# zhaozijie2022/LocoTouch

Measured on AMD Instinct MI355X. Metric: env-steps/sec (whole node), TransportTeacher 4096 envs/GPU, higher is better.
Workload: dtype f32

## Files before the change

### locotouch_amd/_abi.py

```python
from __future__ import annotations

import ctypes
import os
import re

_HERE = os.path.dirname(os.path.abspath(__file__))
REPO = os.path.dirname(_HERE)
HEADER = os.path.join(REPO, "include", "lt_env.h")
OBS_NORM_HEADER = os.path.join(REPO, "include", "lt_obs_norm.h")
STUDENT_HEADER = os.path.join(REPO, "include", "lt_student.h")
COLLECT_HEADER = os.path.join(REPO, "include", "lt_collect.h")
LEDGER_HEADER = os.path.join(REPO, "include", "lt_ledger.h")
CNN_TRAIN_HEADER = os.path.join(REPO, "include", "lt_cnn_train.h")
BC_HEADER = os.path.join(REPO, "include", "lt_bc.h")
LSTM_HEADER = os.path.join(REPO, "include", "lt_lstm.h")
MEMORY_HEADER = os.path.join(REPO, "include", "lt_memory.h")
MEMORY_SEQ_HEADER = os.path.join(REPO, "include", "lt_memory_seq.h")
MEMORY_GRU_HEADER = os.path.join(REPO, "include", "lt_memory_gru.h")
POLICY_HEADER = os.path.join(REPO, "include", "lt_policy.h")
LIB_PATH = os.environ.get("LOCOTOUCH_AMD_LIB", os.path.join(_HERE, "_lib", "liblocotouch_env.so"))

_SCALARS = {"int": ctypes.c_int, "int32_t": ctypes.c_int32, "int64_t": ctypes.c_int64, "uint8_t": ctypes.c_uint8,
            "uint32_t": ctypes.c_uint32, "uint64_t": ctypes.c_uint64, "size_t": ctypes.c_size_t, "float": ctypes.c_float,
            "double": ctypes.c_double}
_DECL = re.compile(r"(?:const\s+)?(\w+)\s*((?:\*\s*(?:const\b\s*)?)*)(\w*)\s*((?:\[[^\]]*\]\s*)*)")


def _ctype(decl, structs, opaque, consts, typed, param):
    m = _DECL.fullmatch(decl.strip())
    if not m:
        return None
    base, stars, name, dims = m.groups()
    depth = stars.count("*")
    try:
        dims = [sum(int(t) if t.strip().isdigit() else consts[t.strip()] for t in d.split("+")) for d in re.findall(r"\[([^\]]*)\]", dims)]
    except KeyError:
        return None
    if param and dims:
        depth, dims = depth + 1, dims[1:]
    t = structs.get(base) or _SCALARS.get(base)
    if (t is None and base not in opaque and base not in ("void", "char")) or depth > 2 or (param and dims):
        return None
    if depth == 0 and t is None:
        return None
    if depth == 1 and base == "char":
        t = ctypes.c_char_p
    elif depth == 1:
        t = ctypes.POINTER(t) if t is not None and (typed or base in structs or base == "size_t") else ctypes.c_void_p
    elif depth == 2:
        t = ctypes.POINTER(ctypes.POINTER(t) if typed and t is not None else ctypes.c_void_p)
    for d in reversed(dims):
        t = t * d
    return name, t


def parse_header(text: str, typed: bool = False, structs: dict | None = None, bases: dict | None = None):
    text = re.sub(r"//[^\n]*", "", re.sub(r"/\*.*?\*/", "", text, flags=re.S))
    consts = {m.group(1): int(m.group(2)) for m in re.finditer(r"#define\s+(LT_\w+)\s+\(?(-?\d+)\)?\s*$", text, flags=re.M)}
    for m in re.finditer(r"enum\s+\w+\s*\{(.*?)\};", text, flags=re.S):
        val = -1
        for item in filter(None, (x.strip() for x in m.group(1).split(","))):
            name, _, v = (x.strip() for x in item.partition("="))
            val = int(v, 0) if v else val + 1
            consts[name] = val
    structs, opaque = dict(structs or {}), set(re.findall(r"typedef\s+struct\s+\w+\s+(\w+)\s*;", text))
    for m in re.finditer(r"typedef\s+struct\s+\w+\s*\{(.*?)\}\s*(\w+)\s*;", text, flags=re.S):
        fields = []
        for line in filter(None, (x.strip() for x in m.group(1).split(";"))):
            first, *more = line.split(",")
            base = _DECL.match(first.strip())
            for decl in [first] + [f"{base.group(1) if base else ''} {x}" for x in more]:
                field = _ctype(decl, structs, opaque, consts, typed, param=False)
                if field is None:
                    raise ImportError(f"cannot type member {decl.strip()!r} of {m.group(2)}")
                fields.append(field)
        pyname = "".join(w.capitalize() for w in m.group(2).split("_"))
        structs[m.group(2)] = type(pyname, ((bases or {}).get(m.group(2), ctypes.Structure),), {"_fields_": fields})
    rest = re.sub(r"^[ \t]*#[^\n]*$|typedef\s+struct\b[^;{]*(\{.*?\})?[^;{]*;|enum\s+\w+\s*\{.*?\};|extern\s+\"C\"\s*\{", "", text, flags=re.S | re.M)
    protos = {}
    for stmt in filter(None, (x.strip() for x in rest.split(";"))):
        m = re.fullmatch(r"(.*?)\b(\w+)\s*\(([^()]*)\)", stmt, flags=re.S)
        if not m:
            if stmt == "}":
                continue
            raise ImportError(f"cannot parse declaration {stmt!r}")
        ret, name, args = m.groups()
        res = (None, None) if ret.strip() == "void" else _ctype(ret, structs, opaque, consts, typed, param=False)
        args = [] if args.strip() == "void" else [_ctype(a, structs, opaque, consts, typed, param=True) for a in args.split(",")]
        if res is None or None in args:
            raise ImportError(f"cannot type prototype {name}: {' '.join(stmt.split())!r}")
        protos[name] = (res[1], [t for _, t in args])
    return consts, structs, protos


class _CfgMethods(ctypes.Structure):
    def copy(self) -> "LtCfg":
        new = LtCfg()
        ctypes.memmove(ctypes.byref(new), ctypes.byref(self), ctypes.sizeof(self))
        for attr in ("extra_reward_terms", "extra_termination_terms", "extra_observation_terms", "reward_term_params"):
            if hasattr(self, attr):
                v = getattr(self, attr)
                setattr(new, attr, dict(v) if isinstance(v, dict) else list(v))
        return new

    def to_dict(self) -> dict:
        def py(v):
            return [py(x) for x in v] if hasattr(v, "__len__") else v

        return {name: py(getattr(self, name)) for name, *_ in self._fields_ if not name.startswith("_")}


CONSTS, STRUCTS, SIGNATURES = parse_header(open(HEADER).read(), bases={"lt_cfg": _CfgMethods})
globals().update(CONSTS)
LtCfg, LtView, LtMlpDesc = STRUCTS["lt_cfg"], STRUCTS["lt_view"], STRUCTS["lt_mlp_desc"]
LtRenderView, LtRenderDesc = STRUCTS["lt_render_view"], STRUCTS["lt_render_desc"]
EXPORTS = list(SIGNATURES)
OBS_NORM_SIGNATURES = parse_header(open(OBS_NORM_HEADER).read())[2]
if any(r is not ctypes.c_int for r, _ in OBS_NORM_SIGNATURES.values()) or set(OBS_NORM_SIGNATURES) & set(EXPORTS):
    raise ImportError("include/lt_obs_norm.h: every entry point returns a status and none repeats one of lt_env.h")

VALUE_QUERIES = frozenset({
    "lt_abi_version", "lt_cfg_sizeof", "lt_cfg_num_presets", "lt_cfg_preset_id", "lt_cfg_obs_dim", "lt_cfg_tactile_dim", "lt_last_error",
    "lt_wgrad_splits", "lt_wgrad_ws_floats", "lt_elu_backward_bias_ws_floats", "lt_head_wgrad_ws_floats", "lt_adam_clip_step_ws_floats",
    "lt_elu_backward_bias_nblk", "lt_head_wgrad_nblk", "lt_mlp_backward_blocks", "lt_env_kernel_name", "lt_mlp_kernel_name"})
if not VALUE_QUERIES <= set(EXPORTS) or any(SIGNATURES[n][0] is not ctypes.c_int for n in set(EXPORTS) - VALUE_QUERIES):
    raise ImportError("_abi.VALUE_QUERIES does not match include/lt_env.h: a query it names is gone, or a new entry point returns no status")

STUDENT_CONSTS, _student_structs, STUDENT_SIGNATURES = parse_header(open(STUDENT_HEADER).read(), structs=STRUCTS)
globals().update(STUDENT_CONSTS)
LtStudentDesc, LtStudentParams = _student_structs["lt_student_desc"], _student_structs["lt_student_params"]
STUDENT_VALUE_QUERIES = frozenset({"lt_student_step_launches"})
if (not STUDENT_VALUE_QUERIES <= set(STUDENT_SIGNATURES) or any(r is not ctypes.c_int for r, _ in STUDENT_SIGNATURES.values())
        or set(STUDENT_SIGNATURES) & (set(EXPORTS) | set(OBS_NORM_SIGNATURES))):
    raise ImportError("_abi.STUDENT_VALUE_QUERIES does not match include/lt_student.h, or an entry point there returns no int or repeats "
                      "one of another header")

COLLECT_SIGNATURES = parse_header(open(COLLECT_HEADER).read())[2]
if (any(r is not ctypes.c_int for r, _ in COLLECT_SIGNATURES.values())
        or set(COLLECT_SIGNATURES) & (set(EXPORTS) | set(OBS_NORM_SIGNATURES) | set(STUDENT_SIGNATURES))):
    raise ImportError("include/lt_collect.h: every entry point returns a status and none repeats one of another header")

LEDGER_CONSTS, _, LEDGER_SIGNATURES = parse_header(open(LEDGER_HEADER).read())
if (any(r is not ctypes.c_int for r, _ in LEDGER_SIGNATURES.values())
        or set(LEDGER_SIGNATURES) & (set(EXPORTS) | set(OBS_NORM_SIGNATURES) | set(STUDENT_SIGNATURES) | set(COLLECT_SIGNATURES))):
    raise ImportError("include/lt_ledger.h: every entry point returns a status and none repeats one of another header")

CNN_TRAIN_CONSTS, _cnn_structs, CNN_TRAIN_SIGNATURES = parse_header(open(CNN_TRAIN_HEADER).read())
globals().update(CNN_TRAIN_CONSTS)
LtCnnDesc, LtCnnParams, LtCnnGrads = _cnn_structs["lt_cnn_desc"], _cnn_structs["lt_cnn_params"], _cnn_structs["lt_cnn_grads"]
CNN_TRAIN_VALUE_QUERIES = frozenset({"lt_cnn_launches"})
if (not CNN_TRAIN_VALUE_QUERIES <= set(CNN_TRAIN_SIGNATURES) or any(r is not ctypes.c_int for r, _ in CNN_TRAIN_SIGNATURES.values())
        or set(CNN_TRAIN_SIGNATURES) & (set(EXPORTS) | set(OBS_NORM_SIGNATURES) | set(STUDENT_SIGNATURES) | set(COLLECT_SIGNATURES)
                                        | set(LEDGER_SIGNATURES))):
    raise ImportError("_abi.CNN_TRAIN_VALUE_QUERIES does not match include/lt_cnn_train.h, or an entry point there returns no int or "
                      "repeats one of another header")

BC_CONSTS, _, BC_SIGNATURES = parse_header(open(BC_HEADER).read())
if (any(r is not ctypes.c_int for r, _ in BC_SIGNATURES.values())
        or set(BC_SIGNATURES) & (set(EXPORTS) | set(OBS_NORM_SIGNATURES) | set(STUDENT_SIGNATURES) | set(COLLECT_SIGNATURES)
                                 | set(LEDGER_SIGNATURES) | set(CNN_TRAIN_SIGNATURES))):
    raise ImportError("include/lt_bc.h: every entry point returns a status and none repeats one of another header")

LSTM_SIGNATURES = parse_header(open(LSTM_HEADER).read())[2]
if (any(r is not ctypes.c_int for r, _ in LSTM_SIGNATURES.values())
        or set(LSTM_SIGNATURES) & (set(EXPORTS) | set(OBS_NORM_SIGNATURES) | set(STUDENT_SIGNATURES) | set(COLLECT_SIGNATURES)
                                   | set(LEDGER_SIGNATURES) | set(CNN_TRAIN_SIGNATURES) | set(BC_SIGNATURES))):
    raise ImportError("include/lt_lstm.h: every entry point returns a status and none repeats one of another header")

_, _memory_structs, MEMORY_SIGNATURES = parse_header(open(MEMORY_HEADER).read())
LtMemoryNet = _memory_structs["lt_memory_net"]
if (any(r is not ctypes.c_int for r, _ in MEMORY_SIGNATURES.values())
        or set(MEMORY_SIGNATURES) & (set(EXPORTS) | set(OBS_NORM_SIGNATURES) | set(STUDENT_SIGNATURES) | set(COLLECT_SIGNATURES)
                                     | set(LEDGER_SIGNATURES) | set(CNN_TRAIN_SIGNATURES) | set(BC_SIGNATURES) | set(LSTM_SIGNATURES))):
    raise ImportError("include/lt_memory.h: every entry point returns a status and none repeats one of another header")

_, _memory_seq_structs, MEMORY_SEQ_SIGNATURES = parse_header(open(MEMORY_SEQ_HEADER).read())
LtMemorySeqNet, LtMemorySeqGrad = _memory_seq_structs["lt_memory_seq_net"], _memory_seq_structs["lt_memory_seq_grad"]
MEMORY_SEQ_VALUE_QUERIES = frozenset({"lt_memory_seq_backward_units"})
if (not MEMORY_SEQ_VALUE_QUERIES <= set(MEMORY_SEQ_SIGNATURES) or any(r is not ctypes.c_int for r, _ in MEMORY_SEQ_SIGNATURES.values())
        or set(MEMORY_SEQ_SIGNATURES) & (set(EXPORTS) | set(OBS_NORM_SIGNATURES) | set(STUDENT_SIGNATURES) | set(COLLECT_SIGNATURES)
                                         | set(LEDGER_SIGNATURES) | set(CNN_TRAIN_SIGNATURES) | set(BC_SIGNATURES) | set(LSTM_SIGNATURES)
                                         | set(MEMORY_SIGNATURES))):
    raise ImportError("_abi.MEMORY_SEQ_VALUE_QUERIES does not match include/lt_memory_seq.h, or an entry point there returns no int or "
                      "repeats one of another header")

_, _memory_gru_structs, MEMORY_GRU_SIGNATURES = parse_header(open(MEMORY_GRU_HEADER).read())
LtMemoryGruNet, LtMemoryGruSeqNet, LtMemoryGruSeqGrad = (_memory_gru_structs[k] for k in ("lt_memory_gru_net", "lt_memory_gru_seq_net",
                                                                                           "lt_memory_gru_seq_grad"))
MEMORY_GRU_VALUE_QUERIES = frozenset({"lt_memory_gru_seq_backward_units"})
if (not MEMORY_GRU_VALUE_QUERIES <= set(MEMORY_GRU_SIGNATURES) or any(r is not ctypes.c_int for r, _ in MEMORY_GRU_SIGNATURES.values())
        or set(MEMORY_GRU_SIGNATURES) & (set(EXPORTS) | set(OBS_NORM_SIGNATURES) | set(STUDENT_SIGNATURES) | set(COLLECT_SIGNATURES)
                                         | set(LEDGER_SIGNATURES) | set(CNN_TRAIN_SIGNATURES) | set(BC_SIGNATURES) | set(LSTM_SIGNATURES)
                                         | set(MEMORY_SIGNATURES) | set(MEMORY_SEQ_SIGNATURES))):
    raise ImportError("_abi.MEMORY_GRU_VALUE_QUERIES does not match include/lt_memory_gru.h, or an entry point there returns no int or "
                      "repeats one of another header")

POLICY_CONSTS, _policy_structs, POLICY_SIGNATURES = parse_header(open(POLICY_HEADER).read(), structs=STRUCTS)
globals().update(POLICY_CONSTS)
LtPolicyDesc, LtPolicyMemory = _policy_structs["lt_policy_desc"], _policy_structs["lt_policy_memory"]
POLICY_VALUE_QUERIES = frozenset({"lt_policy_step_launches"})
if (not POLICY_VALUE_QUERIES <= set(POLICY_SIGNATURES) or any(r is not ctypes.c_int for r, _ in POLICY_SIGNATURES.values())
        or set(POLICY_SIGNATURES) & (set(EXPORTS) | set(OBS_NORM_SIGNATURES) | set(STUDENT_SIGNATURES) | set(COLLECT_SIGNATURES)
                                     | set(LEDGER_SIGNATURES) | set(CNN_TRAIN_SIGNATURES) | set(BC_SIGNATURES) | set(LSTM_SIGNATURES)
                                     | set(MEMORY_SIGNATURES) | set(MEMORY_SEQ_SIGNATURES) | set(MEMORY_GRU_SIGNATURES))):
    raise ImportError("_abi.POLICY_VALUE_QUERIES does not match include/lt_policy.h, or an entry point there returns no int or repeats "
                      "one of another header")

_lib = None
_calls: dict = {}


def load() -> ctypes.CDLL:
    global _lib
    if _lib is not None:
        return _lib
    if not os.path.exists(LIB_PATH):
        raise ImportError(f"{LIB_PATH} is missing: run `python -c 'import __graft_entry__ as g; g.build()'` "
                          "(the HIP extension is mandatory, there is no CPU fallback)")
    lib = ctypes.CDLL(LIB_PATH)
    for name, (restype, argtypes) in {**SIGNATURES, **OBS_NORM_SIGNATURES, **STUDENT_SIGNATURES, **COLLECT_SIGNATURES, **LEDGER_SIGNATURES,
                                      **CNN_TRAIN_SIGNATURES, **BC_SIGNATURES, **LSTM_SIGNATURES, **MEMORY_SIGNATURES,
                                      **MEMORY_SEQ_SIGNATURES, **MEMORY_GRU_SIGNATURES, **POLICY_SIGNATURES}.items():
        fn = getattr(lib, name)
        fn.restype, fn.argtypes = restype, argtypes
        if (name not in VALUE_QUERIES and name not in STUDENT_VALUE_QUERIES and name not in CNN_TRAIN_VALUE_QUERIES
                and name not in MEMORY_SEQ_VALUE_QUERIES and name not in MEMORY_GRU_VALUE_QUERIES and name not in POLICY_VALUE_QUERIES):
            _calls[name] = (fn, [ptr if t is ctypes.c_void_p else _ref if issubclass(t, ctypes._Pointer) and issubclass(t._type_, ctypes.Structure)
                                 else None for t in argtypes])
    if lib.lt_cfg_sizeof() != ctypes.sizeof(LtCfg):
        raise ImportError(f"lt_cfg ABI mismatch: C {lib.lt_cfg_sizeof()} vs ctypes {ctypes.sizeof(LtCfg)}")
    if lib.lt_abi_version() != CONSTS["LT_ABI_VERSION"]:
        raise ImportError("lt_env.h / liblocotouch_env.so ABI version mismatch")
    _lib = lib
    return lib


def ptr(x):
    if x is None or isinstance(x, int):
        return ctypes.c_void_p(x or None)
    data_ptr = getattr(x, "data_ptr", None)
    return ctypes.c_void_p(data_ptr()) if data_ptr else x


def _ref(x):
    return ctypes.byref(x) if isinstance(x, ctypes.Structure) else x


def stream(device=None) -> ctypes.c_void_p:
    import torch

    return ctypes.c_void_p(torch.cuda.current_stream(device).cuda_stream)


def ptr_array(tensors):
    return (ctypes.c_void_p * max(1, len(tensors)))(*[None if t is None else t.data_ptr() for t in tensors])


def call(name: str, *args) -> None:
    try:
        fn, conv = _calls[name]
    except KeyError:
        if (name in VALUE_QUERIES or name in STUDENT_VALUE_QUERIES or name in CNN_TRAIN_VALUE_QUERIES or name in MEMORY_SEQ_VALUE_QUERIES
                or name in MEMORY_GRU_VALUE_QUERIES or name in POLICY_VALUE_QUERIES):
            raise TypeError(f"{name} returns a value, not a status: call load().{name}(...)") from None
        if _lib is not None:
            raise
        load()
        fn, conv = _calls[name]
    rc = fn(*[a if c is None else c(a) for c, a in zip(conv, args, strict=True)])
    if rc:
        check(rc, name)


def preset_ids() -> list[str]:
    lib = load()
    return [lib.lt_cfg_preset_id(i).decode() for i in range(lib.lt_cfg_num_presets())]


def preset_cfg(gym_id: str, num_envs: int | None = None, seed: int | None = None) -> LtCfg:
    cfg = LtCfg()
    rc = load().lt_cfg_preset(gym_id.encode(), ctypes.byref(cfg))
    if rc != 0:
        raise KeyError(f"unknown task {gym_id!r}; registered: {preset_ids()}")
    if num_envs is not None:
        cfg.num_envs = int(num_envs)
    if seed is not None:
        cfg.seed = int(seed)
    return cfg


def default_cfg(task: int, num_envs: int | None = None, seed: int | None = None) -> LtCfg:
    cfg = LtCfg()
    rc = load().lt_cfg_default(task, ctypes.byref(cfg))
    if rc != 0:
        raise ValueError(f"lt_cfg_default({task}) failed: {rc}")
    if num_envs is not None:
        cfg.num_envs = num_envs
    if seed is not None:
        cfg.seed = seed
    return cfg


def check(rc: int, what: str) -> None:
    if rc != 0:
        err = load().lt_last_error()
        raise RuntimeError(f"{what} failed with code {rc}: {err.decode() if err else ''}")
```

### locotouch_amd/csrc/lt_ppo.hip

```cpp
#include <hip/hip_runtime.h>
#include <math.h>
#include <stdint.h>

#include "lt_env.h"
#include "lt_internal.h"

namespace {

constexpr int MAX_A = 16;
constexpr float kHalfLog2Pi = 0.91893853320467274178f;

__global__ __launch_bounds__(256) void lt_ppo_loss_kernel(const float* __restrict__ mu, const float* __restrict__ stdp, const float* __restrict__ value,
                                                          const float* __restrict__ actions, const float* __restrict__ old_logp,
                                                          const float* __restrict__ adv, const float* __restrict__ returns,
                                                          const float* __restrict__ old_values, const float* __restrict__ old_mu,
                                                          const float* __restrict__ old_sigma, const long long* __restrict__ idx,
                                                          long long M, int A, float clip, float vcoef, int clipped_value,
                                                          float* __restrict__ dmu, float* __restrict__ dvalue, float* __restrict__ acc) {
  const long long row = (long long)blockIdx.x * 256 + threadIdx.x;
  const bool ok = row < M;
  const long long src = (ok && idx) ? idx[row] : row;
  float part[4 + MAX_A];
  float amax_mu = 0.f, amax_v = 0.f;
#pragma unroll
  for (int i = 0; i < 4 + MAX_A; ++i) part[i] = 0.f;
  if (ok) {
    const float inv_m = 1.f / (float)M;
    float logp = 0.f, kl = 0.f;
    float z[MAX_A], isg[MAX_A];
#pragma unroll
    for (int a = 0; a < MAX_A; ++a) {
      if (a < A) {
        const float sg = stdp[a], m = mu[row * A + a], x = actions[src * A + a];
        const float om = old_mu[src * A + a], os = old_sigma[src * A + a];
        isg[a] = 1.f / sg;
        z[a] = (x - m) * isg[a];
        logp += -0.5f * z[a] * z[a] - __logf(sg) - kHalfLog2Pi;
        {
#pragma clang fp reciprocal(off)
          kl += logf(sg / os + 1.0e-5f) + (os * os + (om - m) * (om - m)) / (2.f * sg * sg) - 0.5f;
        }
      }
    }
    const float advr = adv[src];
    const float ratio = __expf(logp - old_logp[src]);
    const float s1 = -advr * ratio;
    const float rc = fminf(fmaxf(ratio, 1.f - clip), 1.f + clip);
    const float s2 = -advr * rc;
    const bool inside = ratio >= 1.f - clip && ratio <= 1.f + clip;
    const float dsurr_dratio = (s1 > s2 || inside) ? -advr : 0.f;
    const float dlogp = dsurr_dratio * ratio * inv_m;
#pragma unroll
    for (int a = 0; a < MAX_A; ++a) {
      if (a < A) {
        dmu[row * A + a] = dlogp * z[a] * isg[a];
        amax_mu = fmaxf(amax_mu, fabsf(dlogp * z[a] * isg[a]));
        part[4 + a] = dlogp * (z[a] * z[a] - 1.f) * isg[a];
      }
    }
    const float v = value[row], R = returns[src];
    float vl, dv;
    if (clipped_value) {
      const float ov = old_values[src];
      const float dcl = fminf(fmaxf(v - ov, -clip), clip);
      const float vc = ov + dcl;
      const float l1 = (v - R) * (v - R), l2 = (vc - R) * (vc - R);
      const bool in_v = (v - ov) >= -clip && (v - ov) <= clip;
      vl = fmaxf(l1, l2);
      dv = (l1 > l2 || in_v) ? 2.f * (v - R) : 0.f;
    } else {
      vl = (R - v) * (R - v);
      dv = 2.f * (v - R);
    }
    dvalue[row] = vcoef * dv * inv_m;
    amax_v = fabsf(vcoef * dv * inv_m);
    part[0] = fmaxf(s1, s2);
    part[1] = vl;
    part[2] = kl;
  }
  __shared__ float red[4][4 + MAX_A];
  const int lane = threadIdx.x & 63, wave = threadIdx.x >> 6;
#pragma unroll
  for (int i = 0; i < 4 + MAX_A; ++i) {
    float v = part[i];
#pragma unroll
    for (int off = 32; off > 0; off >>= 1) v += __shfl_xor(v, off, 64);
    if (lane == 0) red[wave][i] = v;
  }
#pragma unroll
  for (int off = 32; off > 0; off >>= 1) {
    amax_mu = fmaxf(amax_mu, __shfl_xor(amax_mu, off, 64));
    amax_v = fmaxf(amax_v, __shfl_xor(amax_v, off, 64));
  }
  __shared__ float redm[4][2];
  if (lane == 0) { redm[wave][0] = amax_mu; redm[wave][1] = amax_v; }
  __syncthreads();
  if (threadIdx.x < 4 + A && threadIdx.x != 3) {
    const int i = threadIdx.x;
    atomicAdd(acc + i, red[0][i] + red[1][i] + red[2][i] + red[3][i]);
  } else if (threadIdx.x >= 64 && threadIdx.x < 66) {
    const int j = threadIdx.x - 64;
    atomicMax((unsigned*)acc + 20 + j, __float_as_uint(fmaxf(fmaxf(redm[0][j], redm[1][j]), fmaxf(redm[2][j], redm[3][j]))));
  }
}

__global__ __launch_bounds__(64) void lt_ppo_finalize_kernel(const float* __restrict__ acc, const float* __restrict__ stdp, int A, float inv_m,
                                                             float vcoef, float ecoef, float* __restrict__ out) {
  const int a = threadIdx.x;
  float e = 0.f;
  if (a < A) {
    const float sg = stdp[a];
    e = 0.5f + kHalfLog2Pi + logf(sg);
    out[8 + a] = acc[4 + a] - ecoef / sg;
  }
  for (int off = 32; off > 0; off >>= 1) e += __shfl_xor(e, off, 64);
  if (a == 0) {
    const float surr = acc[0] * inv_m, vl = acc[1] * inv_m;
    out[0] = surr + vcoef * vl - ecoef * e;
    out[1] = surr; out[2] = vl; out[3] = e; out[4] = acc[2] * inv_m;
  }
}

constexpr int EB_ROWS = 48;

__global__ __launch_bounds__(256) void lt_elu_bwd_bias_kernel(const float* da, const float* __restrict__ a, long long M, int N, float alpha,
                                                              float* dz, float* __restrict__ ws, float* __restrict__ amax) {
  const int n4 = N >> 2, lanes = 256 / n4;
  const int c4 = threadIdx.x % n4, rl = threadIdx.x / n4;
  const long long r0 = (long long)blockIdx.x * EB_ROWS;
  float4 sum = {0.f, 0.f, 0.f, 0.f};
  float mx = 0.f;
  if (rl < lanes) {
    for (int r = rl; r < EB_ROWS; r += lanes) {
      const long long row = r0 + r;
      if (row >= M) break;
      const float4 g = ((const float4*)(da + row * N))[c4], y = ((const float4*)(a + row * N))[c4];
      float4 o;
      o.x = g.x * (y.x > 0.f ? 1.f : y.x + alpha);
      o.y = g.y * (y.y > 0.f ? 1.f : y.y + alpha);
      o.z = g.z * (y.z > 0.f ? 1.f : y.z + alpha);
      o.w = g.w * (y.w > 0.f ? 1.f : y.w + alpha);
      ((float4*)(dz + row * N))[c4] = o;
      sum.x += o.x; sum.y += o.y; sum.z += o.z; sum.w += o.w;
      mx = fmaxf(fmaxf(mx, fmaxf(fabsf(o.x), fabsf(o.y))), fmaxf(fabsf(o.z), fabsf(o.w)));
    }
  }
  __shared__ float4 red[256];
  __shared__ float redm[4];
  red[threadIdx.x] = sum;
  if (amax) {
#pragma unroll
    for (int off = 32; off > 0; off >>= 1) mx = fmaxf(mx, __shfl_xor(mx, off, 64));
    if ((threadIdx.x & 63) == 0) redm[threadIdx.x >> 6] = mx;
  }
  __syncthreads();
  if (amax && threadIdx.x == 0) amax[blockIdx.x] = fmaxf(fmaxf(redm[0], redm[1]), fmaxf(redm[2], redm[3]));
  if (threadIdx.x < n4) {
    float4 t = red[threadIdx.x];
    for (int l = 1; l < lanes; ++l) {
      const float4 u = red[l * n4 + threadIdx.x];
      t.x += u.x; t.y += u.y; t.z += u.z; t.w += u.w;
    }
    ((float4*)(ws + (long long)blockIdx.x * N))[threadIdx.x] = t;
  }
}

constexpr int SUM_MAX_JOBS = 24;
struct SumJobs {
  const float* ws[SUM_MAX_JOBS];
  float* out0[SUM_MAX_JOBS];
  float* out1[SUM_MAX_JOBS];
  long long stride[SUM_MAX_JOBS];
  int nblk[SUM_MAX_JOBS], count[SUM_MAX_JOBS], split[SUM_MAX_JOBS], first[SUM_MAX_JOBS + 1];
  int njobs;
};
__host__ __device__ inline int sum_row_lanes(int nblk) { return nblk >= 96 ? 16 : 4; }

__global__ __launch_bounds__(256) void lt_partial_sums_kernel(const SumJobs J) {
  const int ln = (int)threadIdx.x & 63;
  const int f = (ln >= 1 && ln < J.njobs) ? J.first[ln] : 0x7fffffff;
  const int j = __builtin_amdgcn_readfirstlane((int)__popcll(__ballot(f <= (int)blockIdx.x)));
  const float* __restrict__ ws = J.ws[j];
  const int nblk = J.nblk[j], count = J.count[j], split = J.split[j];
  const long long stride = J.stride[j];
  const int RL = sum_row_lanes(nblk), cols = 256 / RL;
  const int c = (int)threadIdx.x % cols, lane = (int)threadIdx.x / cols;
  const int e = ((int)blockIdx.x - J.first[j]) * cols * 4 + 4 * c;
  const bool vec = e + 3 < count && ((stride & 3) == 0) && ((reinterpret_cast<uintptr_t>(ws) & 15) == 0);
  float4 s[4];
#pragma unroll
  for (int u = 0; u < 4; ++u) s[u] = make_float4(0.f, 0.f, 0.f, 0.f);
  if (e < count) {
    auto at = [&](int b) __attribute__((always_inline)) {
      const float* p = ws + (long long)b * stride + e;
      if (vec) return *(const float4*)p;
      return make_float4(p[0], e + 1 < count ? p[1] : 0.f, e + 2 < count ? p[2] : 0.f, e + 3 < count ? p[3] : 0.f);
    };
    int b = lane;
    for (; b + 3 * RL < nblk; b += 4 * RL) {
#pragma unroll
      for (int u = 0; u < 4; ++u) {
        const float4 v = at(b + u * RL);
        s[u].x += v.x; s[u].y += v.y; s[u].z += v.z; s[u].w += v.w;
      }
    }
#pragma unroll
    for (int u = 0; u < 3; ++u) {
      if (b < nblk) {
        const float4 v = at(b);
        s[u].x += v.x; s[u].y += v.y; s[u].z += v.z; s[u].w += v.w;
        b += RL;
      }
    }
  }
  __shared__ float4 red[256];
  red[threadIdx.x] = make_float4((s[0].x + s[1].x) + (s[2].x + s[3].x), (s[0].y + s[1].y) + (s[2].y + s[3].y),
                                 (s[0].z + s[1].z) + (s[2].z + s[3].z), (s[0].w + s[1].w) + (s[2].w + s[3].w));
  __syncthreads();
  if (lane == 0 && e < count) {
    float4 t = red[c];
    for (int l = 1; l < RL; ++l) { const float4 v = red[l * cols + c]; t.x += v.x; t.y += v.y; t.z += v.z; t.w += v.w; }
    const float o[4] = {t.x, t.y, t.z, t.w};
#pragma unroll
    for (int i = 0; i < 4; ++i) {
      const int ei = e + i;
      if (ei >= count) break;
      if (ei < split) J.out0[j][ei] = o[i];
      else if (J.out1[j]) J.out1[j][ei - split] = o[i];
    }
  }
}

void launch_one_sum(const float* ws, int nblk, long long stride, int count, int split, float* out0, float* out1, hipStream_t stream) {
  SumJobs J = {};
  J.njobs = 1;
  J.ws[0] = ws; J.out0[0] = out0; J.out1[0] = out1; J.stride[0] = stride;
  J.nblk[0] = nblk; J.count[0] = count; J.split[0] = split;
  const int epb = 256 / sum_row_lanes(nblk) * 4;
  J.first[1] = (count + epb - 1) / epb;
  hipLaunchKernelGGL(lt_partial_sums_kernel, dim3((unsigned)J.first[1]), dim3(256), 0, stream, J);
}

constexpr int HW_ROWS = 96, HW_MAX_N = 16;

template <int NN>
__global__ __launch_bounds__(256) void lt_head_wgrad_kernel(const float* __restrict__ dy, const float* __restrict__ x, int x_split, long long M, int n, int k,
                                                            float* __restrict__ ws) {
  const int k4 = k >> 2, lanes = 256 / k4;
  const int c4 = threadIdx.x % k4, rl = threadIdx.x / k4;
  const long long r0 = (long long)blockIdx.x * HW_ROWS;
  float4 acc[NN];
  float accb[NN];
#pragma unroll
  for (int j = 0; j < NN; ++j) { acc[j] = {0.f, 0.f, 0.f, 0.f}; accb[j] = 0.f; }
  if (rl < lanes) {
    for (int r = rl; r < HW_ROWS; r += 4 * lanes) {
      float4 xv[4];
      float d[4][NN];
#pragma unroll
      for (int u = 0; u < 4; ++u) {
        const long long row = r0 + r + u * lanes;
        const bool ok = (r + u * lanes) < HW_ROWS && row < M;
        xv[u] = ok ? ((const float4*)(x + row * k))[c4] : float4{0.f, 0.f, 0.f, 0.f};
        if (x_split) {
          const unsigned w[4] = {__float_as_uint(xv[u].x), __float_as_uint(xv[u].y), __float_as_uint(xv[u].z), __float_as_uint(xv[u].w)};
          float f[4];
#pragma unroll
          for (int i = 0; i < 4; ++i)
            f[i] = (float)__builtin_bit_cast(_Float16, (unsigned short)(w[i] & 0xFFFFu)) + (float)__builtin_bit_cast(_Float16, (unsigned short)(w[i] >> 16)) * (1.f / 64.f);
          xv[u] = float4{f[0], f[1], f[2], f[3]};
        }
#pragma unroll
        for (int j = 0; j < NN; ++j) d[u][j] = (ok && j < n) ? dy[row * n + j] : 0.f;
      }
#pragma unroll
      for (int u = 0; u < 4; ++u)
#pragma unroll
        for (int j = 0; j < NN; ++j) {
          acc[j].x += d[u][j] * xv[u].x; acc[j].y += d[u][j] * xv[u].y; acc[j].z += d[u][j] * xv[u].z; acc[j].w += d[u][j] * xv[u].w;
          accb[j] += d[u][j];
        }
    }
  }
  extern __shared__ float4 red[];
  float* const redb = (float*)(red + (size_t)lanes * NN * k4);
  if (rl < lanes) {
#pragma unroll
    for (int j = 0; j < NN; ++j) red[((size_t)rl * NN + j) * k4 + c4] = acc[j];
    if (c4 == 0)
#pragma unroll
      for (int j = 0; j < NN; ++j) redb[rl * NN + j] = accb[j];
  }
  __syncthreads();
  float* const out = ws + (size_t)blockIdx.x * ((size_t)n * k + HW_MAX_N);
  for (int e = threadIdx.x; e < n * k4; e += 256) {
    const int j = e / k4, c = e - j * k4;
    float4 t = red[(size_t)j * k4 + c];
    for (int l = 1; l < lanes; ++l) {
      const float4 u = red[((size_t)l * NN + j) * k4 + c];
      t.x += u.x; t.y += u.y; t.z += u.z; t.w += u.w;
    }
    ((float4*)(out + (size_t)j * k))[c] = t;
  }
  if (threadIdx.x < n) {
    float t = redb[threadIdx.x];
    for (int l = 1; l < lanes; ++l) t += redb[l * NN + threadIdx.x];
    out[(size_t)n * k + threadIdx.x] = t;
  }
}

__global__ __launch_bounds__(256) void lt_gae_kernel(const float* __restrict__ rewards, const unsigned char* __restrict__ dones,
                                                     const float* __restrict__ values, const float* __restrict__ last_values, float gamma,
                                                     float lam, int T, long long N, float* __restrict__ returns, float* __restrict__ advantages) {
  const long long e = (long long)blockIdx.x * 256 + threadIdx.x;
  if (e >= N) return;
  float next_v = last_values[e], gae = 0.f;
  for (int t = T - 1; t >= 0; --t) {
    const long long o = (long long)t * N + e;
    const float v = values[o], alive = 1.f - (float)dones[o];
    const float delta = rewards[o] + alive * gamma * next_v - v;
    gae = delta + alive * gamma * lam * gae;
    const float ret = gae + v;
    returns[o] = ret;
    advantages[o] = ret - v;
    next_v = v;
  }
}

constexpr int AD_PER_BLOCK = 2048;

__global__ __launch_bounds__(256) void lt_sumsq_kernel(const float* __restrict__ g, long long n, float* __restrict__ ws) {
  const long long base = (long long)blockIdx.x * AD_PER_BLOCK;
  float s = 0.f;
  for (int k = threadIdx.x; k < AD_PER_BLOCK; k += 256) {
    const long long i = base + k;
    if (i < n) s += g[i] * g[i];
  }
  for (int off = 32; off > 0; off >>= 1) s += __shfl_xor(s, off, 64);
  __shared__ float red[4];
  if ((threadIdx.x & 63) == 0) red[threadIdx.x >> 6] = s;
  __syncthreads();
  if (threadIdx.x == 0) ws[blockIdx.x] = (red[0] + red[1]) + (red[2] + red[3]);
}

__global__ __launch_bounds__(256) void lt_adam_kernel(float* __restrict__ p, float* __restrict__ g, float* __restrict__ m, float* __restrict__ v,
                                                      long long n, const float* __restrict__ ws, int nblk, float max_norm, float b1,
                                                      float b2, float eps, float wd, float step_size, float bc2_sqrt, float* __restrict__ norm_out,
                                                      const float* __restrict__ lr_dev, float inv_bc1) {
  __shared__ float s_coef;
  if (lr_dev) step_size = *lr_dev * inv_bc1;
  if (threadIdx.x < 64) {
    float s = 0.f;
    for (int b = threadIdx.x; b < nblk; b += 64) s += ws[b];
    for (int off = 32; off > 0; off >>= 1) s += __shfl_xor(s, off, 64);
    if (threadIdx.x == 0) {
      const float norm = sqrtf(s);
      const float c = max_norm / (norm + 1.0e-6f);
      s_coef = max_norm > 0.f ? (c < 1.f ? c : 1.f) : 1.f;
      if (blockIdx.x == 0 && norm_out) *norm_out = norm;
    }
  }
  __syncthreads();
  const float coef = s_coef;
  const long long base = (long long)blockIdx.x * AD_PER_BLOCK;
  for (int k = threadIdx.x; k < AD_PER_BLOCK; k += 256) {
    const long long i = base + k;
    if (i >= n) break;
    float gi = g[i] * coef;
    g[i] = gi;
    const float pi = p[i];
    if (wd != 0.f) gi += wd * pi;
    const float mi = m[i] + (1.f - b1) * (gi - m[i]);
    const float vi = b2 * v[i] + (1.f - b2) * gi * gi;
    m[i] = mi;
    v[i] = vi;
    p[i] = pi - step_size * (mi / (sqrtf(vi) / bc2_sqrt + eps));
  }
}

__global__ __launch_bounds__(64) void lt_ppo_lr_rule_kernel(const float* __restrict__ kl_mean, float desired, float lr_min, float lr_max, float factor,
                                                            float* __restrict__ lr, float* __restrict__ stats, const float* __restrict__ scalars,
                                                            float* __restrict__ dstd_out, int A) {
  if (dstd_out && scalars && (int)threadIdx.x < A) dstd_out[threadIdx.x] = scalars[8 + threadIdx.x];
  if (threadIdx.x != 0) return;
  if (kl_mean && desired > 0.f) {
#pragma clang fp reciprocal(off)
    const float kl = *kl_mean;
    float v = *lr;
    if (kl > desired * 2.f) v = fmaxf(lr_min, v / factor);
    else if (kl < desired * 0.5f && kl > 0.f) v = fminf(lr_max, v * factor);
    *lr = v;
  }
  if (stats && scalars) { stats[0] += scalars[2]; stats[1] += scalars[1]; stats[2] += scalars[3]; }
}

}

extern "C" int lt_ppo_lr_rule(const float* kl_mean, float desired_kl, float lr_min, float lr_max, float factor, float* lr, float* stats,
                              const float* scalars, float* dstd_out, int num_actions, void* stream) {
  if (!lr || factor <= 1.f || num_actions < 0 || num_actions > MAX_A) { lt_set_error("lt_ppo_lr_rule: invalid argument"); return LT_EINVAL; }
  hipLaunchKernelGGL(lt_ppo_lr_rule_kernel, dim3(1), dim3(64), 0, (hipStream_t)stream, kl_mean, desired_kl, lr_min, lr_max, factor, lr, stats, scalars,
                     dstd_out, num_actions);
  const hipError_t e = hipGetLastError();
  if (e != hipSuccess) { lt_set_error(hipGetErrorString(e)); return LT_EHIP; }
  return LT_OK;
}

static int elu_backward_bias(const float* da, const float* a, int64_t M, int N, float alpha, float* dz, float* db, float* ws, float* amax, void* stream);
extern "C" int lt_elu_backward_bias(const float* da, const float* a, int64_t M, int N, float alpha, float* dz, float* db, float* ws, void* stream) {
  return elu_backward_bias(da, a, M, N, alpha, dz, db, ws, nullptr, stream);
}
extern "C" int lt_elu_backward_bias2(const float* da, const float* a, int64_t M, int N, float alpha, float* dz, float* db, float* ws, float* amax_blocks,
                                     void* stream) {
  return elu_backward_bias(da, a, M, N, alpha, dz, db, ws, amax_blocks, stream);
}
static int elu_backward_bias(const float* da, const float* a, int64_t M, int N, float alpha, float* dz, float* db, float* ws, float* amax, void* stream) {
  if (!da || !a || !dz || !ws || M < 1 || N < 4 || (N & 3) || N > 1024) {
    lt_set_error("lt_elu_backward_bias: invalid argument (N a multiple of 4, 4 <= N <= 1024)");
    return LT_EINVAL;
  }
  const int nblk = (int)((M + EB_ROWS - 1) / EB_ROWS);
  hipLaunchKernelGGL(lt_elu_bwd_bias_kernel, dim3((unsigned)nblk), dim3(256), 0, (hipStream_t)stream, da, a, (long long)M, N, alpha, dz, ws, amax);
  if (db) launch_one_sum(ws, nblk, (long long)N, N, N, db, nullptr, (hipStream_t)stream);
  const hipError_t e = hipGetLastError();
  if (e != hipSuccess) { lt_set_error(hipGetErrorString(e)); return LT_EHIP; }
  return LT_OK;
}

extern "C" int64_t lt_head_wgrad_ws_floats(int64_t M, int n, int k) { return ((M + HW_ROWS - 1) / HW_ROWS) * ((int64_t)n * k + HW_MAX_N); }

extern "C" int lt_head_wgrad(const float* dy, const float* x, int x_split, int64_t M, int n, int k, float* dw, float* db, float* ws, void* stream) {
  if (!dy || !x || !ws || M < 1 || n < 1 || n > HW_MAX_N || k < 4 || (k & 3) || k > 1024) {
    lt_set_error("lt_head_wgrad: invalid argument (1 <= n <= 16, k a multiple of 4, 4 <= k <= 1024)");
    return LT_EINVAL;
  }
  const int nblk = (int)((M + HW_ROWS - 1) / HW_ROWS), k4 = k / 4, lanes = 256 / k4;
  const int nn = n <= 1 ? 1 : (n <= 4 ? 4 : (n <= 8 ? 8 : (n <= 12 ? 12 : 16)));
  const size_t lds = (size_t)lanes * nn * k4 * 16 + (size_t)lanes * nn * 4;
  if (const int e = lt_ensure_dynamic_lds((const void*)lt_head_wgrad_kernel<16>, 72 * 1024)) {
    lt_set_error(hipGetErrorString((hipError_t)e));
    return LT_EHIP;
  }
  if (lds > 72 * 1024) {
    lt_set_error("lt_head_wgrad: n * k too large for one block's LDS partials");
    return LT_EINVAL;
  }
  const dim3 g((unsigned)nblk), b(256);
  hipStream_t st = (hipStream_t)stream;
  switch (nn) {
    case 1: hipLaunchKernelGGL(lt_head_wgrad_kernel<1>, g, b, lds, st, dy, x, x_split, (long long)M, n, k, ws); break;
    case 4: hipLaunchKernelGGL(lt_head_wgrad_kernel<4>, g, b, lds, st, dy, x, x_split, (long long)M, n, k, ws); break;
    case 8: hipLaunchKernelGGL(lt_head_wgrad_kernel<8>, g, b, lds, st, dy, x, x_split, (long long)M, n, k, ws); break;
    case 12: hipLaunchKernelGGL(lt_head_wgrad_kernel<12>, g, b, lds, st, dy, x, x_split, (long long)M, n, k, ws); break;
    default: hipLaunchKernelGGL(lt_head_wgrad_kernel<16>, g, b, lds, st, dy, x, x_split, (long long)M, n, k, ws); break;
  }
  if (dw) launch_one_sum(ws, nblk, (long long)n * k + HW_MAX_N, n * k + n, n * k, dw, db, st);
  const hipError_t e = hipGetLastError();
  if (e != hipSuccess) { lt_set_error(hipGetErrorString(e)); return LT_EHIP; }
  return LT_OK;
}

extern "C" int lt_partial_sums(int njobs, const float* const* ws, const int* nblk, const int64_t* stride, const int* count, const int* split,
                               float* const* out0, float* const* out1, void* stream) {
  if (njobs < 1 || njobs > SUM_MAX_JOBS || !ws || !nblk || !stride || !count || !split || !out0 || !out1) {
    lt_set_error("lt_partial_sums: invalid argument (1 <= njobs <= 24)");
    return LT_EINVAL;
  }
  SumJobs J = {};
  J.njobs = njobs;
  int blocks = 0;
  for (int j = 0; j < njobs; ++j) {
    if (!ws[j] || !out0[j] || nblk[j] < 1 || count[j] < 1) { lt_set_error("lt_partial_sums: invalid job"); return LT_EINVAL; }
    J.ws[j] = ws[j]; J.out0[j] = out0[j]; J.out1[j] = out1[j]; J.stride[j] = stride[j];
    J.nblk[j] = nblk[j]; J.count[j] = count[j]; J.split[j] = split[j];
    J.first[j] = blocks;
    const int epb = 256 / sum_row_lanes(nblk[j]) * 4;
    blocks += (count[j] + epb - 1) / epb;
  }
  J.first[njobs] = blocks;
  hipLaunchKernelGGL(lt_partial_sums_kernel, dim3((unsigned)blocks), dim3(256), 0, (hipStream_t)stream, J);
  const hipError_t e = hipGetLastError();
  if (e != hipSuccess) { lt_set_error(hipGetErrorString(e)); return LT_EHIP; }
  return LT_OK;
}
extern "C" int lt_elu_backward_bias_nblk(int64_t M) { return (int)((M + EB_ROWS - 1) / EB_ROWS); }
extern "C" int lt_head_wgrad_nblk(int64_t M) { return (int)((M + HW_ROWS - 1) / HW_ROWS); }

extern "C" int lt_gae(const float* rewards, const uint8_t* dones, const float* values, const float* last_values, float gamma, float lam, int T,
                      int64_t N, float* returns, float* advantages, void* stream) {
  if (!rewards || !dones || !values || !last_values || !returns || !advantages || T < 1 || N < 1) {
    lt_set_error("lt_gae: invalid argument");
    return LT_EINVAL;
  }
  hipLaunchKernelGGL(lt_gae_kernel, dim3((unsigned)((N + 255) / 256)), dim3(256), 0, (hipStream_t)stream, rewards, dones, values, last_values, gamma,
                     lam, T, (long long)N, returns, advantages);
  const hipError_t e = hipGetLastError();
  if (e != hipSuccess) { lt_set_error(hipGetErrorString(e)); return LT_EHIP; }
  return LT_OK;
}

extern "C" int64_t lt_elu_backward_bias_ws_floats(int64_t M, int N) { return ((M + EB_ROWS - 1) / EB_ROWS) * (int64_t)N; }

static int adam_clip_step(float* params, float* grads, float* exp_avg, float* exp_avg_sq, int64_t n, float max_norm, float lr, const float* lr_dev,
                          float beta1, float beta2, float eps, float weight_decay, int64_t step, float* ws, float* grad_norm, void* stream);

extern "C" int lt_adam_clip_step(float* params, float* grads, float* exp_avg, float* exp_avg_sq, int64_t n, float max_norm, float lr, float beta1,
                                 float beta2, float eps, float weight_decay, int64_t step, float* ws, float* grad_norm, void* stream) {
  return adam_clip_step(params, grads, exp_avg, exp_avg_sq, n, max_norm, lr, nullptr, beta1, beta2, eps, weight_decay, step, ws, grad_norm, stream);
}

extern "C" int lt_adam_clip_step_dev(float* params, float* grads, float* exp_avg, float* exp_avg_sq, int64_t n, float max_norm, const float* lr_dev,
                                     float beta1, float beta2, float eps, float weight_decay, int64_t step, float* ws, float* grad_norm, void* stream) {
  if (!lr_dev) { lt_set_error("lt_adam_clip_step_dev: null learning-rate pointer"); return LT_EINVAL; }
  return adam_clip_step(params, grads, exp_avg, exp_avg_sq, n, max_norm, 0.f, lr_dev, beta1, beta2, eps, weight_decay, step, ws, grad_norm, stream);
}

static int adam_clip_step(float* params, float* grads, float* exp_avg, float* exp_avg_sq, int64_t n, float max_norm, float lr, const float* lr_dev,
                          float beta1, float beta2, float eps, float weight_decay, int64_t step, float* ws, float* grad_norm, void* stream) {
  if (!params || !grads || !exp_avg || !exp_avg_sq || !ws || n < 1 || step < 1) {
    lt_set_error("lt_adam_clip_step: invalid argument");
    return LT_EINVAL;
  }
  const int nblk = (int)((n + AD_PER_BLOCK - 1) / AD_PER_BLOCK);
  const double bc1 = 1.0 - pow((double)beta1, (double)step), bc2 = 1.0 - pow((double)beta2, (double)step);
  hipLaunchKernelGGL(lt_sumsq_kernel, dim3((unsigned)nblk), dim3(256), 0, (hipStream_t)stream, grads, (long long)n, ws);
  hipLaunchKernelGGL(lt_adam_kernel, dim3((unsigned)nblk), dim3(256), 0, (hipStream_t)stream, params, grads, exp_avg, exp_avg_sq, (long long)n, ws, nblk,
                     max_norm, beta1, beta2, eps, weight_decay, (float)((double)lr / bc1), (float)sqrt(bc2), grad_norm, lr_dev, (float)(1.0 / bc1));
  const hipError_t e = hipGetLastError();
  if (e != hipSuccess) { lt_set_error(hipGetErrorString(e)); return LT_EHIP; }
  return LT_OK;
}

extern "C" int64_t lt_adam_clip_step_ws_floats(int64_t n) { return (n + AD_PER_BLOCK - 1) / AD_PER_BLOCK; }

extern "C" int lt_ppo_loss(const float* mu, const float* stdp, const float* value, const float* actions, const float* old_logp, const float* adv,
                           const float* returns, const float* old_values, const float* old_mu, const float* old_sigma, const int64_t* idx,
                           int64_t M, int A, float clip, float value_loss_coef, float entropy_coef, int use_clipped_value_loss, float* dmu, float* dvalue,
                           float* acc, float* out, void* stream) {
  if (!mu || !stdp || !value || !actions || !old_logp || !adv || !returns || !old_values || !old_mu || !old_sigma || !dmu || !dvalue || !acc ||
      M < 1 || A < 1 || A > MAX_A) {
    lt_set_error("lt_ppo_loss: invalid argument (1 <= num_actions <= 16)");
    return LT_EINVAL;
  }
  hipError_t e = hipMemsetAsync(acc, 0, sizeof(float) * (4 + MAX_A + 4), (hipStream_t)stream);
  if (e != hipSuccess) { lt_set_error(hipGetErrorString(e)); return LT_EHIP; }
  hipLaunchKernelGGL(lt_ppo_loss_kernel, dim3((unsigned)((M + 255) / 256)), dim3(256), 0, (hipStream_t)stream, mu, stdp, value, actions, old_logp, adv,
                     returns, old_values, old_mu, old_sigma, (const long long*)idx, (long long)M, A, clip, value_loss_coef, use_clipped_value_loss, dmu, dvalue, acc);
  if (out) hipLaunchKernelGGL(lt_ppo_finalize_kernel, dim3(1), dim3(64), 0, (hipStream_t)stream, acc, stdp, A, 1.f / (float)M, value_loss_coef, entropy_coef, out);
  e = hipGetLastError();
  if (e != hipSuccess) { lt_set_error(hipGetErrorString(e)); return LT_EHIP; }
  return LT_OK;
}
```

### locotouch_amd/csrc/lt_wgrad.hip

```cpp
#include <hip/hip_runtime.h>
#include <stdint.h>

#include "lt_env.h"
#include "lt_internal.h"

namespace {

typedef float f32x4 __attribute__((ext_vector_type(4)));
typedef float f32x2 __attribute__((ext_vector_type(2)));
typedef _Float16 f16x8 __attribute__((ext_vector_type(8)));
typedef _Float16 f16x2 __attribute__((ext_vector_type(2)));

constexpr int TA = 4, TB = 4;
constexpr float LO_SCALE = 64.f;

template <int U>
__device__ __forceinline__ void split8(const f32x4 (&v)[8], float scale, f16x8& hi, f16x8& lo) {
#pragma unroll
  for (int p = 0; p < 4; ++p) {
    f32x2 x;
    x[0] = v[2 * p][U] * scale; x[1] = v[2 * p + 1][U] * scale;
    const f16x2 h = __builtin_convertvector(x, f16x2);
    const f32x2 d = (x - __builtin_convertvector(h, f32x2)) * LO_SCALE;
    const f16x2 l = __builtin_convertvector(d, f16x2);
    hi[2 * p] = h[0]; hi[2 * p + 1] = h[1];
    lo[2 * p] = l[0]; lo[2 * p + 1] = l[1];
  }
}

template <int U>
__device__ __forceinline__ void unpack8(const f32x4 (&v)[8], f16x8& hi, f16x8& lo) {
  typedef unsigned u32x4 __attribute__((ext_vector_type(4)));
  u32x4 h, l;
#pragma unroll
  for (int p = 0; p < 4; ++p) {
    const unsigned w0 = __float_as_uint(v[2 * p][U]), w1 = __float_as_uint(v[2 * p + 1][U]);
    h[p] = __builtin_amdgcn_perm(w1, w0, 0x05040100u);
    l[p] = __builtin_amdgcn_perm(w1, w0, 0x07060302u);
  }
  hi = __builtin_bit_cast(f16x8, h);
  lo = __builtin_bit_cast(f16x8, l);
}

struct WgradArgs {
  const float* dz;
  const float* x;
  long long M;
  int N, K;
  int tiles_n, tiles_k, splits;
  const float* amax;
  int nblk_amax;
  float* slabs;
  int dz_split;
  const float* dz_scale;
  int x_split;
  float* db;
};

constexpr int WG_WAVES = 4;
template <bool AS, bool XS>
__global__ __launch_bounds__(64 * WG_WAVES, 2) void lt_wgrad_kernel(const WgradArgs a) {
  __shared__ f32x4 s_tile[WG_WAVES - 1][TA * TB + 1][64];
  const int lane = threadIdx.x & 63;
  const int wave = __builtin_amdgcn_readfirstlane((int)threadIdx.x >> 6);
  const int i = lane & 15, g = lane >> 4;
  const int tiles = a.tiles_n * a.tiles_k;
  const int per_xcd = (int)gridDim.x >> 3;
  const int item = ((int)blockIdx.x & 7) * per_xcd + ((int)blockIdx.x >> 3);
  if (item >= tiles * a.splits) return;
  const int split = item / tiles, tile = item - split * tiles;
  const int tn = tile / a.tiles_k, tk = tile - tn * a.tiles_k;
  const int n0 = tn * 16 * TA, k0 = tk * 16 * TB;
  const long long steps = (a.M + 31) / 32;
  const long long b0 = steps * split / a.splits, b1 = steps * (split + 1) / a.splits;
  const long long s0 = b0 + (b1 - b0) * wave / WG_WAVES, s1 = b0 + (b1 - b0) * (wave + 1) / WG_WAVES;
  float scale = 1.f;
  if (AS) {
    scale = *a.dz_scale;
  } else if (a.amax) {
    float m = 0.f;
    for (int b = lane; b < a.nblk_amax; b += 64) m = fmaxf(m, a.amax[b]);
#pragma unroll
    for (int off = 32; off > 0; off >>= 1) m = fmaxf(m, __shfl_xor(m, off, 64));
    const int e = (int)((__float_as_uint(m) >> 23) & 0xFF) - 127;
    int se = 7 - e;
    se = se > 100 ? 100 : (se < -100 ? -100 : se);
    scale = __uint_as_float((unsigned)(127 + se) << 23);
  }
  f32x4 acc[TA][TB];
#pragma unroll
  for (int p = 0; p < TA; ++p)
#pragma unroll
    for (int q = 0; q < TB; ++q) acc[p][q] = f32x4{0.f, 0.f, 0.f, 0.f};
  f32x4 va[8], vb[8];
  const int ca = min(n0 + 4 * i, a.N - 4), cb = min(k0 + 4 * i, a.K - 4);
  const unsigned row_a = (unsigned)a.N * 4u, row_b = (unsigned)a.K * 4u;
  const unsigned last_a = (unsigned)(a.M - 1) * row_a + (unsigned)ca * 4u, last_b = (unsigned)(a.M - 1) * row_b + (unsigned)cb * 4u;
  unsigned off_a = ((unsigned)s0 * 32u + (unsigned)g) * row_a + (unsigned)ca * 4u, off_b = ((unsigned)s0 * 32u + (unsigned)g) * row_b + (unsigned)cb * 4u;
  auto issue = [&](long long) __attribute__((always_inline)) {
#pragma unroll
    for (int t = 0; t < 8; ++t) {
      va[t] = *(const f32x4*)((const char*)a.dz + min(off_a + (unsigned)(4 * t) * row_a, last_a));
      vb[t] = *(const f32x4*)((const char*)a.x + min(off_b + (unsigned)(4 * t) * row_b, last_b));
    }
    off_a += 32u * row_a;
    off_b += 32u * row_b;
  };
  const bool colsum = a.db != nullptr && tk == 0;
  f32x4 cs = f32x4{0.f, 0.f, 0.f, 0.f};
  if (s0 < s1) issue(s0);
  for (long long s = s0; s < s1; ++s) {
    if ((s + 1) * 32 > a.M) {
#pragma unroll
      for (int t = 0; t < 8; ++t) if (s * 32 + 4 * t + g >= a.M) va[t] = f32x4{0.f, 0.f, 0.f, 0.f};
    }
    if (colsum) {
      if (AS) {
#pragma unroll
        for (int t = 0; t < 8; ++t)
#pragma unroll
          for (int u = 0; u < 4; ++u) {
            const unsigned w = __float_as_uint(va[t][u]);
            cs[u] += (float)__builtin_bit_cast(_Float16, (unsigned short)(w & 0xFFFFu)) + (float)__builtin_bit_cast(_Float16, (unsigned short)(w >> 16)) * (1.f / LO_SCALE);
          }
      } else {
#pragma unroll
        for (int t = 0; t < 8; ++t) cs += va[t];
      }
    }
    f16x8 ah[TA], al[TA], bh[TB], bl[TB];
    if (AS) {
      unpack8<0>(va, ah[0], al[0]); unpack8<1>(va, ah[1], al[1]); unpack8<2>(va, ah[2], al[2]); unpack8<3>(va, ah[3], al[3]);
    } else {
      split8<0>(va, scale, ah[0], al[0]); split8<1>(va, scale, ah[1], al[1]); split8<2>(va, scale, ah[2], al[2]); split8<3>(va, scale, ah[3], al[3]);
    }
    if (XS) {
      unpack8<0>(vb, bh[0], bl[0]); unpack8<1>(vb, bh[1], bl[1]); unpack8<2>(vb, bh[2], bl[2]); unpack8<3>(vb, bh[3], bl[3]);
    } else {
      split8<0>(vb, 1.f, bh[0], bl[0]); split8<1>(vb, 1.f, bh[1], bl[1]); split8<2>(vb, 1.f, bh[2], bl[2]); split8<3>(vb, 1.f, bh[3], bl[3]);
    }
    if (s + 1 < s1) issue(s + 1);
#pragma unroll
    for (int p = 0; p < TA; ++p) {
      const f16x8 a64 = ah[p] * (_Float16)LO_SCALE;
#pragma unroll
      for (int q = 0; q < TB; ++q) {
        acc[p][q] = __builtin_amdgcn_mfma_f32_16x16x32_f16(a64, bh[q], acc[p][q], 0, 0, 0);
        acc[p][q] = __builtin_amdgcn_mfma_f32_16x16x32_f16(ah[p], bl[q], acc[p][q], 0, 0, 0);
        acc[p][q] = __builtin_amdgcn_mfma_f32_16x16x32_f16(al[p], bh[q], acc[p][q], 0, 0, 0);
      }
    }
  }
  if (wave > 0) {
#pragma unroll
    for (int p = 0; p < TA; ++p)
#pragma unroll
      for (int q = 0; q < TB; ++q) s_tile[wave - 1][p * TB + q][lane] = acc[p][q];
    s_tile[wave - 1][TA * TB][lane] = cs;
  }
  __syncthreads();
  if (wave > 0) return;
#pragma unroll
  for (int w = 0; w < WG_WAVES - 1; ++w) {
#pragma unroll
    for (int p = 0; p < TA; ++p)
#pragma unroll
      for (int q = 0; q < TB; ++q) acc[p][q] += s_tile[w][p * TB + q][lane];
    cs += s_tile[w][TA * TB][lane];
  }
  if (colsum) {
#pragma unroll
    for (int u = 0; u < 4; ++u) {
      cs[u] += __shfl_xor(cs[u], 16, 64);
      cs[u] += __shfl_xor(cs[u], 32, 64);
    }
    if (AS) cs *= 1.f / scale;
    if (g == 0 && n0 + 4 * i < a.N) *(f32x4*)(a.db + (long long)split * a.N + n0 + 4 * i) = cs;
  }
  const float inv = 1.f / (scale * LO_SCALE);
  float* const out = a.slabs + (long long)split * a.N * a.K;
  const int k = k0 + 4 * i;
#pragma unroll
  for (int p = 0; p < TA; ++p)
#pragma unroll
    for (int r = 0; r < 4; ++r) {
      const int n = n0 + 4 * (4 * g + r) + p;
      if (n < a.N && k < a.K) {
        f32x4 o;
#pragma unroll
        for (int q = 0; q < TB; ++q) o[q] = acc[p][q][r] * inv;
        *(f32x4*)(out + (long long)n * a.K + k) = o;
      }
    }
}

int pick_splits(long long M, int tiles) {
  const long long steps = (M + 31) / 32;
  long long s = 512 / tiles;
  if (s > steps / 8) s = steps / 8;
  return (int)(s < 1 ? 1 : s);
}

}

extern "C" int lt_wgrad_splits(int64_t M, int N, int K) {
  const int tiles = ((N + 16 * TA - 1) / (16 * TA)) * ((K + 16 * TB - 1) / (16 * TB));
  return pick_splits((long long)M, tiles);
}

extern "C" int64_t lt_wgrad_ws_floats(int64_t M, int N, int K) { return (int64_t)lt_wgrad_splits(M, N, K) * N * K; }

extern "C" int lt_wgrad(const float* dz, int dz_split, const float* dz_scale, const float* x, int x_split, int64_t M, int N, int K, const float* amax_blocks,
                        int nblk_amax, float* slabs, float* db_slabs, void* stream) {
  if (!dz || !x || !slabs || M < 1 || N < 4 || K < 4 || (N & 3) || (K & 3) || (amax_blocks && nblk_amax < 1) || (long long)M * (N > K ? N : K) * 4 >= (1ll << 32)) {
    lt_set_error("lt_wgrad: invalid argument (N and K multiples of 4, each operand below 4 GiB)");
    return LT_EINVAL;
  }
  WgradArgs a;
  a.dz = dz; a.x = x; a.M = M; a.N = N; a.K = K;
  a.amax = amax_blocks; a.nblk_amax = amax_blocks ? nblk_amax : 0;
  a.slabs = slabs; a.db = db_slabs; a.x_split = x_split != 0; a.dz_split = dz_split != 0; a.dz_scale = dz_scale;
  if (a.dz_split && !dz_scale) { lt_set_error("lt_wgrad: a split dz needs its scale"); return LT_EINVAL; }
  a.tiles_n = (N + 16 * TA - 1) / (16 * TA);
  a.tiles_k = (K + 16 * TB - 1) / (16 * TB);
  a.splits = pick_splits((long long)M, a.tiles_n * a.tiles_k);
  const dim3 grid((unsigned)((a.tiles_n * a.tiles_k * a.splits + 7) / 8 * 8));
  if (a.dz_split && a.x_split) hipLaunchKernelGGL((lt_wgrad_kernel<true, true>), grid, dim3(64 * WG_WAVES), 0, (hipStream_t)stream, a);
  else if (a.x_split) hipLaunchKernelGGL((lt_wgrad_kernel<false, true>), grid, dim3(64 * WG_WAVES), 0, (hipStream_t)stream, a);
  else if (a.dz_split) hipLaunchKernelGGL((lt_wgrad_kernel<true, false>), grid, dim3(64 * WG_WAVES), 0, (hipStream_t)stream, a);
  else hipLaunchKernelGGL((lt_wgrad_kernel<false, false>), grid, dim3(64 * WG_WAVES), 0, (hipStream_t)stream, a);
  const hipError_t e = hipGetLastError();
  if (e != hipSuccess) { lt_set_error(hipGetErrorString(e)); return LT_EHIP; }
  return LT_OK;
}

namespace {
__global__ __launch_bounds__(256) void lt_split_rows_kernel(const float* __restrict__ x, unsigned* __restrict__ out, long long n4) {
  typedef unsigned u32x4 __attribute__((ext_vector_type(4)));
  const long long i = (long long)blockIdx.x * 256 + threadIdx.x;
  if (i >= n4) return;
  const f32x4 v = ((const f32x4*)x)[i];
  u32x4 o;
#pragma unroll
  for (int k = 0; k < 4; ++k) {
    const float c = __builtin_amdgcn_fmed3f(v[k], -(float)LT_MLP_INPUT_CLAMP, (float)LT_MLP_INPUT_CLAMP);
    const _Float16 h = (_Float16)c;
    const _Float16 l = (_Float16)((c - (float)h) * LO_SCALE);
    o[k] = (unsigned)__builtin_bit_cast(unsigned short, h) | ((unsigned)__builtin_bit_cast(unsigned short, l) << 16);
  }
  ((u32x4*)out)[i] = o;
}
}

extern "C" int lt_split_rows(const float* x, void* out, int64_t count, void* stream) {
  if (!x || !out || count < 4 || (count & 3)) { lt_set_error("lt_split_rows: invalid argument (count a multiple of 4)"); return LT_EINVAL; }
  hipLaunchKernelGGL(lt_split_rows_kernel, dim3((unsigned)((count / 4 + 255) / 256)), dim3(256), 0, (hipStream_t)stream, x, (unsigned*)out, (long long)(count / 4));
  const hipError_t e = hipGetLastError();
  if (e != hipSuccess) { lt_set_error(hipGetErrorString(e)); return LT_EHIP; }
  return LT_OK;
}
```

### locotouch_amd/rl/mlp.py

```python
from __future__ import annotations

import ctypes
import os

import torch
import torch.nn as nn

from .. import _abi

USE_FUSED_BACKWARD = os.environ.get("LT_FUSED_BACKWARD", "1") != "0"
_ACT_IDS = {nn.ELU: "LT_ACT_ELU", nn.ReLU: "LT_ACT_RELU", nn.Tanh: "LT_ACT_TANH", nn.Identity: "LT_ACT_NONE"}


def describe(seq: nn.Sequential):
    linears, acts = [], set()
    mods = list(seq)
    for i, m in enumerate(mods):
        if isinstance(m, nn.Linear):
            if m.bias is None or m.weight.dtype != torch.float32:
                return None
            linears.append(m)
        elif type(m) in _ACT_IDS:
            if type(m) is nn.ELU and (m.alpha != 1.0):
                return None
            if i == 0 or not isinstance(mods[i - 1], nn.Linear) or i == len(mods) - 1:
                return None
            acts.add(type(m))
        else:
            return None
    C = _abi.CONSTS
    if not linears or len(linears) > C["LT_MLP_MAX_LAYERS"] or len(acts) > 1:
        return None
    if len(linears) > 1 and len(mods) != 2 * len(linears) - 1:
        return None
    dims = [linears[0].in_features] + [l.out_features for l in linears]
    if dims[0] > C["LT_MLP_MAX_WIDTH"] or any(d > 512 for d in dims[1:]):
        return None
    if any(a.out_features != b.in_features for a, b in zip(linears[:-1], linears[1:])):
        return None
    desc = _abi.LtMlpDesc()
    desc.num_layers = len(linears)
    for i, d in enumerate(dims):
        desc.dims[i] = d
    desc.activation = C[_ACT_IDS[next(iter(acts))]] if acts else C["LT_ACT_NONE"]
    return desc, linears


class PackedMLP:
    def __init__(self, seq: nn.Sequential):
        got = describe(seq)
        if got is None:
            raise ValueError("network shape not supported by lt_mlp_forward (Linear/activation stack, hidden widths <= 512)")
        self.desc, self.linears = got
        self.lib = _abi.load()
        n = ctypes.c_size_t()
        _abi.call("lt_mlp_packed_floats", self.desc, ctypes.byref(n))
        dev = self.linears[0].weight.device
        self.packed = torch.zeros(n.value, device=dev, dtype=torch.float32)
        self.bpacked = None
        self.in_dtype = torch.float32
        self.out_features = self.linears[-1].out_features
        self.in_features = self.linears[0].in_features
        self.pack()

    def weight_ptrs(self):
        return _abi.ptr_array([l.weight for l in self.linears])

    def bias_ptrs(self):
        return _abi.ptr_array([l.bias for l in self.linears])

    def pack(self) -> None:
        for l in self.linears:
            if not l.weight.is_contiguous():
                raise ValueError("Linear.weight must be contiguous")
        _abi.call("lt_mlp_pack", self.desc, self.weight_ptrs(), self.bias_ptrs(), self.packed, _abi.stream())

    def backward_ok(self) -> bool:
        n = ctypes.c_size_t()
        return self.lib.lt_mlp_backward_packed_floats(ctypes.byref(self.desc), ctypes.byref(n)) == 0

    def alloc_bpacked(self) -> None:
        if self.bpacked is None:
            n = ctypes.c_size_t()
            _abi.call("lt_mlp_backward_packed_floats", self.desc, ctypes.byref(n))
            self.bpacked = torch.zeros(n.value, device=self.packed.device, dtype=torch.float32)

    def pack_backward(self) -> None:
        self.alloc_bpacked()
        _abi.call("lt_mlp_pack_backward", self.desc, self.weight_ptrs(), self.bpacked, _abi.stream())

    def set_input_format(self, dtype: torch.dtype) -> None:
        if dtype not in (torch.float32, torch.bfloat16):
            raise ValueError("input rows are float32 or bfloat16")
        if dtype == torch.bfloat16 and self.in_features % 4:
            raise ValueError("bfloat16 input rows need in_features % 4 == 0")
        self.desc.input_format = _abi.CONSTS["LT_ROWS_BF16"] if dtype == torch.bfloat16 else _abi.CONSTS["LT_ROWS_F32"]
        self.in_dtype = dtype

    def forward(self, x: torch.Tensor, out: torch.Tensor | None = None) -> torch.Tensor:
        if x.dim() != 2 or x.shape[1] != self.in_features or x.dtype != self.in_dtype or not x.is_contiguous():
            raise ValueError("x must be a contiguous [m, in_features] tensor of the input format")
        m = x.shape[0]
        if out is None:
            out = torch.empty(m, self.out_features, device=x.device, dtype=torch.float32)
        _abi.call("lt_mlp_forward", self.desc, self.packed, x, m, out, _abi.stream())
        return out

    __call__ = forward


def _alloc_outputs(nets, m, device):
    ys, acts = [], []
    for net in nets:
        dims = [net.desc.dims[i] for i in range(net.desc.num_layers + 1)]
        ys.append(torch.empty(m, dims[-1], device=device, dtype=torch.float32))
        acts.append([torch.empty(m, d, device=device, dtype=torch.float32) for d in dims[1:-1]])
    return ys, acts


def _forward_pair(nets, x0, x1, acts_split: bool):
    ys, acts = _alloc_outputs(nets, x0.shape[0], x0.device)
    _abi.call("lt_mlp_forward_pair", nets[0].desc, nets[0].packed, x0, nets[1].desc, nets[1].packed, x1, x0.shape[0], ys[0], ys[1],
              _abi.ptr_array(acts[0]), _abi.ptr_array(acts[1]), int(acts_split), _abi.stream())
    return ys, acts


class _PairForward(torch.autograd.Function):

    @staticmethod
    def forward(ctx, pair, x0, x1, *params):
        nets = (pair.a, pair.b)
        ys, acts = _forward_pair(nets, x0, x1, acts_split=False)
        if pair.check_domain:
            pair._record_domain((x0, x1, *acts[0], *acts[1]))
        ctx.nl = (len(nets[0].linears), len(nets[1].linears))
        ctx.save_for_backward(x0, x1, *acts[0], *acts[1], *[p for p in params[0::2]])
        ctx.elu = nets[0].desc.activation == _abi.CONSTS["LT_ACT_ELU"]
        return ys[0], ys[1]

    @staticmethod
    def backward(ctx, dy0, dy1):
        from .linear import _head_wgrad, _head_wgrad_ok, _wgrad, pick_splits

        lib = _abi.load()
        saved = list(ctx.saved_tensors)
        x = saved[:2]
        n0, n1 = ctx.nl
        acts = [saved[2:2 + n0 - 1], saved[2 + n0 - 1:2 + n0 - 1 + n1 - 1]]
        ws = saved[2 + n0 - 1 + n1 - 1:]
        weights = [ws[:n0], ws[n0:]]
        grads = []
        for k, dy in enumerate((dy0, dy1)):
            L = len(weights[k])
            g = dy if dy.is_contiguous() else dy.contiguous()
            layer_grads = [None] * (2 * L)
            for l in range(L - 1, -1, -1):
                inp = acts[k][l - 1] if l > 0 else x[k]
                w = weights[k][l]
                m, n = g.shape
                if l < L - 1:
                    a = acts[k][l]
                    dz = torch.empty_like(a)
                    db = torch.empty(n, device=a.device, dtype=torch.float32)
                    scratch = torch.empty(lib.lt_elu_backward_bias_ws_floats(m, n), device=a.device, dtype=torch.float32)
                    _abi.call("lt_elu_backward_bias", g, a, m, n, 1.0, dz, db, scratch, _abi.stream())
                    dw = _wgrad(dz, inp, pick_splits(m, n, inp.shape[1]))
                else:
                    dz = g
                    if _head_wgrad_ok(dz, inp):
                        dw, db = _head_wgrad(dz, inp)
                    else:
                        dw, db = _wgrad(dz, inp, pick_splits(m, n, inp.shape[1])), dz.sum(0)
                layer_grads[2 * l], layer_grads[2 * l + 1] = dw, db
                if l > 0:
                    g = dz @ w
            grads += layer_grads
        return (None, None, None, *grads)


class SumJobs:

    MAX = 24

    def __init__(self):
        self.jobs: list = []
        self.after: list = []

    def add(self, ws, nblk, stride, count, split, out0, out1=None) -> None:
        self.jobs.append((ws, int(nblk), int(stride), int(count), int(split), out0, out1))

    def launch(self) -> None:
        while self.jobs:
            batch, self.jobs = self.jobs[:self.MAX], self.jobs[self.MAX:]
            n = len(batch)
            ws, nblk, stride, count, split, out0, out1 = zip(*batch)
            _abi.call("lt_partial_sums", n, _abi.ptr_array(ws), (ctypes.c_int * n)(*nblk), (ctypes.c_int64 * n)(*stride),
                      (ctypes.c_int * n)(*count), (ctypes.c_int * n)(*split), _abi.ptr_array(out0), _abi.ptr_array(out1), _abi.stream())
            self._keep = batch
        for dst, src in self.after:
            dst.copy_(src)
        self.after = []


def backward_chain(weights, biases_out, weights_out, x, acts, dy, sums: SumJobs):
    from .linear import _head_wgrad_ok, pick_splits

    lib = _abi.load()
    stream = _abi.stream()
    L = len(weights)
    g = dy if dy.is_contiguous() else dy.contiguous()
    for l in range(L - 1, -1, -1):
        inp = acts[l - 1] if l > 0 else x
        w = weights[l]
        m, n = g.shape
        k = inp.shape[1]
        if l < L - 1:
            a = acts[l]
            dz = torch.empty_like(a)
            nblk = lib.lt_elu_backward_bias_nblk(m)
            scratch = torch.empty(nblk * n + nblk, device=a.device, dtype=torch.float32)
            amax = scratch[nblk * n:]
            _abi.call("lt_elu_backward_bias2", g, a, m, n, 1.0, dz, None, scratch, amax, stream)
            sums.add(scratch, nblk, n, n, n, biases_out[l])
        else:
            dz, amax = g, None
        if l == L - 1 and _head_wgrad_ok(dz, inp):
            nblk = lib.lt_head_wgrad_nblk(m)
            ws = torch.empty(lib.lt_head_wgrad_ws_floats(m, n, k), device=inp.device, dtype=torch.float32)
            _abi.call("lt_head_wgrad", dz, inp, 0, m, n, k, None, None, ws, stream)
            sums.add(ws, nblk, n * k + 16, n * k + n, n * k, weights_out[l], biases_out[l])
        elif amax is not None and n % 4 == 0 and k % 4 == 0:
            sp = lib.lt_wgrad_splits(m, n, k)
            slabs = torch.empty(sp * n * k, device=inp.device, dtype=torch.float32)
            _abi.call("lt_wgrad", dz, 0, None, inp, 0, m, n, k, amax, amax.numel(), slabs, None, stream)
            sums.add(slabs, sp, n * k, n * k, n * k, weights_out[l])
        else:
            sp = pick_splits(m, n, k)
            if sp > 1:
                slabs = torch.bmm(dz.view(sp, m // sp, n).transpose(1, 2), inp.view(sp, m // sp, k))
                sums.add(slabs, sp, n * k, n * k, n * k, weights_out[l])
            else:
                torch.mm(dz.t(), inp, out=weights_out[l])
            if l == L - 1:
                torch.sum(dz, dim=0, out=biases_out[l])
        if l > 0:
            g = dz @ w


class PackedPair:

    def __init__(self, actor: nn.Sequential, critic: nn.Sequential):
        self.a, self.b = PackedMLP(actor), PackedMLP(critic)
        self.check_domain = False
        self.domain_max: torch.Tensor | None = None
        self.acts_split = False
        self._bpacked_fresh = False
        self._bwd_shapes_ok: bool | None = None
        self.sat: torch.Tensor | None = None
        for net in (self.a, self.b):
            dims = [net.desc.dims[i] for i in range(net.desc.num_layers + 1)]
            if any(d % 4 for d in dims[1:-1]) or net.desc.activation != _abi.CONSTS["LT_ACT_ELU"]:
                raise ValueError("PackedPair: ELU stacks with hidden widths that are multiples of 4")

    def arm_domain_check(self) -> None:
        self.check_domain = True

    def _record_domain(self, tensors) -> None:
        self.check_domain = False
        with torch.no_grad():
            m_ = torch.stack([t.abs().max().float() for t in tensors]).max()
            self.domain_max = m_ if self.domain_max is None else torch.maximum(self.domain_max, m_)

    def domain_violated(self) -> bool:
        if self.domain_max is None:
            return False
        v = float(self.domain_max)
        self.domain_max = None
        return v >= float(_abi.CONSTS["LT_MLP_INPUT_CLAMP"])

    def forward_raw(self, x0: torch.Tensor, x1: torch.Tensor, split: bool | None = None):
        if split is None:
            split = self._fused_backward_possible(x0, x1)
        self.acts_split = bool(split)
        self.pack_training(with_backward=self.acts_split)
        ys, acts = _forward_pair((self.a, self.b), x0, x1, self.acts_split)
        if self.check_domain:
            hidden = [t.view(torch.float16)[:, 0::2] if self.acts_split else t for t in (*acts[0], *acts[1])]
            self._record_domain((x0, x1, *hidden))
        return ys, acts

    def pack_training(self, with_backward: bool) -> None:
        args = []
        for net in (self.a, self.b):
            if with_backward:
                net.alloc_bpacked()
            args += [net.desc, net.weight_ptrs(), net.bias_ptrs(), net.packed, net.bpacked if with_backward else None]
        _abi.call("lt_mlp_pack_training", *args, _abi.stream())
        self._bpacked_fresh = bool(with_backward)

    def split_rows(self, x: torch.Tensor) -> torch.Tensor:
        k = x.shape[1]
        if k % 4:
            xp = torch.zeros(x.shape[0], k + (-k) % 4, device=x.device, dtype=torch.float32)
            xp[:, :k] = x
            x = xp
        out = torch.empty_like(x, dtype=torch.float32)
        _abi.call("lt_split_rows", x, out, x.numel(), _abi.stream())
        return out

    def _fused_backward_possible(self, x0, x1) -> bool:
        from .linear import _head_wgrad_ok

        if not USE_FUSED_BACKWARD:
            return False
        if x0.dtype != torch.float32 or x1.dtype != torch.float32 or not x0.is_contiguous() or not x1.is_contiguous():
            return False
        if self._bwd_shapes_ok is None:
            ok = self.a.backward_ok() and self.b.backward_ok()
            for net in (self.a, self.b):
                dims = [net.desc.dims[i] for i in range(net.desc.num_layers + 1)]
                ok = ok and dims[0] % 2 == 0
                ok = ok and _head_wgrad_ok(torch.empty(0, dims[-1], device=x0.device), torch.empty(0, dims[-2], device=x0.device))
            self._bwd_shapes_ok = bool(ok)
        return self._bwd_shapes_ok

    def _fused_backward_ok(self, x0, x1, dy0, dy1) -> bool:
        return self._fused_backward_possible(x0, x1) and dy0.dtype == torch.float32 and dy1.dtype == torch.float32

    def _backward_fused(self, x0, x1, acts, dy0, dy1, grad_of, sums, x_split_rows=None, after_first=None, dy_amax=None) -> None:
        lib = _abi.load()
        stream = _abi.stream()
        m = x0.shape[0]
        nets, xs = (self.a, self.b), (x0, x1)
        asp = int(self.acts_split)
        xsp = int(x_split_rows is not None)
        if not xsp and any(x.shape[1] % 4 for x in xs):
            x_split_rows, xsp = (self.split_rows(x0), self.split_rows(x1)), 1
        if xsp:
            xs = x_split_rows
        dys = [d if d.is_contiguous() else d.contiguous() for d in (dy0, dy1)]
        dev = x0.device
        if self.sat is None:
            self.sat = torch.zeros(1, device=dev, dtype=torch.float32)
        nblk = lib.lt_mlp_backward_blocks(ctypes.byref(nets[0].desc), ctypes.byref(nets[1].desc), m)
        dzs, amaxs, arrs = [], [], []
        per_net = (SumJobs(), SumJobs()) if after_first is not None else (sums, sums)
        for k, net in enumerate(nets):
            if not self._bpacked_fresh:
                net.pack_backward()
            L = len(net.linears)
            n, kk = dys[k].shape[1], acts[k][L - 2].shape[1]
            ws = torch.empty(lib.lt_head_wgrad_ws_floats(m, n, kk), device=dev, dtype=torch.float32)
            _abi.call("lt_head_wgrad", dys[k], acts[k][L - 2], asp, m, n, kk, None, None, ws, stream)
            per_net[k].add(ws, lib.lt_head_wgrad_nblk(m), n * kk + 16, n * kk + n, n * kk, grad_of[net.linears[L - 1].weight], grad_of[net.linears[L - 1].bias])
            dz = [torch.empty_like(a) for a in acts[k]]
            am = torch.empty(L - 1, nblk, device=dev, dtype=torch.float32)
            dzs.append(dz)
            amaxs.append(am)
            arrs.append((_abi.ptr_array(acts[k]), _abi.ptr_array(dz), _abi.ptr_array([am[l] for l in range(L - 1)])))
        dzsp = int(dy_amax is not None)
        scales = torch.empty(2, device=dev, dtype=torch.float32)
        in_amax = dy_amax if dzsp else (None, None)
        _abi.call("lt_mlp_backward_pair", nets[0].desc, nets[0].bpacked, dys[0], *arrs[0], nets[1].desc, nets[1].bpacked, dys[1], *arrs[1],
                  m, asp, in_amax[0], in_amax[1], dzsp, scales, self.sat, stream)
        for k, net in enumerate(nets):
            for l in range(len(net.linears) - 2, -1, -1):
                inp = acts[k][l - 1] if l > 0 else xs[k]
                dz = dzs[k][l]
                n, kk = dz.shape[1], inp.shape[1]
                sp = lib.lt_wgrad_splits(m, n, kk)
                slabs = torch.empty(sp * n * kk + sp * n, device=dev, dtype=torch.float32)
                dbs = slabs[sp * n * kk:]
                _abi.call("lt_wgrad", dz, dzsp, scales[k:k + 1], inp, asp if l > 0 else xsp, m, n, kk, amaxs[k][l], nblk, slabs, dbs, stream)
                gw = grad_of[net.linears[l].weight]
                if kk != gw.shape[1]:
                    pad = torch.empty(n, kk, device=dev, dtype=torch.float32)
                    per_net[k].add(slabs, sp, n * kk, n * kk, n * kk, pad)
                    per_net[k].after.append((gw, pad[:, :gw.shape[1]]))
                else:
                    per_net[k].add(slabs, sp, n * kk, n * kk, n * kk, gw)
                per_net[k].add(dbs, sp, n, n, n, grad_of[net.linears[l].bias])
            if after_first is not None:
                per_net[k].launch()
                if k == 0:
                    after_first()
        self._keep_bwd = (dzs, amaxs, dys, per_net, scales if dzsp else None)
        self._bpacked_fresh = False

    def saturated(self) -> torch.Tensor | None:
        return self.sat

    def backward_raw(self, x0, x1, acts, dy0, dy1, grad_of, x_split_rows=None, after_first=None, dy_amax=None) -> None:
        sums = SumJobs()
        if self._fused_backward_ok(x0, x1, dy0, dy1):
            self._backward_fused(x0, x1, acts, dy0, dy1, grad_of, sums, x_split_rows, after_first, dy_amax)
            sums.launch()
            return
        if self.acts_split:
            raise RuntimeError("PackedPair.backward_raw: the activations are in the split format, which only the fused backward pass reads "
                               "(forward_raw(..., split=False) for the library path)")
        for net, x, a, dy in ((self.a, x0, acts[0], dy0), (self.b, x1, acts[1], dy1)):
            ws = [lin.weight for lin in net.linears]
            backward_chain(ws, [grad_of[lin.bias] for lin in net.linears], [grad_of[lin.weight] for lin in net.linears], x, a, dy, sums)
        sums.launch()

    def __call__(self, x0: torch.Tensor, x1: torch.Tensor):
        self.a.pack()
        self.b.pack()
        params = []
        for net in (self.a, self.b):
            for lin in net.linears:
                params += [lin.weight, lin.bias]
        return _PairForward.apply(self, x0.contiguous(), x1.contiguous(), *params)
```

### locotouch_amd/rl/ppo.py

```python
from __future__ import annotations

import torch
import torch.nn as nn

from .. import _abi
from .dist import Dist
from .modules import ActorCritic
from .storage import RolloutStorage


class PPO:
    def __init__(self, actor_critic: ActorCritic, num_learning_epochs=1, num_mini_batches=1, clip_param=0.2, gamma=0.998,
                 lam=0.95, value_loss_coef=1.0, entropy_coef=0.0, learning_rate=1e-3, max_grad_norm=1.0,
                 use_clipped_value_loss=True, schedule="fixed", desired_kl=0.01, device="cpu",
                 normalize_advantage_per_mini_batch=False, dist: Dist | None = None, **unused):
        self.device = device
        self.dist = dist or Dist()
        self.actor_critic = actor_critic.to(device)
        on_gpu = torch.device(device).type == "cuda"
        self.fused_loss = on_gpu and bool(unused.get("fused_loss", True))
        self.packed_forward = on_gpu and bool(unused.get("packed_forward", True))
        self.direct_update = on_gpu and bool(unused.get("direct_update", True))
        self.fused_recurrent_update = bool(unused.get("fused_recurrent_update", False))
        self.fused_gru_memories = bool(unused.get("fused_gru_memories", False))
        if self.fused_recurrent_update:
            why = self._recurrent_update_unsupported()
            if why is not None:
                raise ValueError(f"fused_recurrent_update: {why}")
        self._pair = None
        if on_gpu and bool(unused.get("tuned_gemms", True)):
            from . import tuned_gemms

            tuned_gemms.enable()
        self.optimizer = torch.optim.Adam(self.actor_critic.parameters(), lr=learning_rate)
        self.storage: RolloutStorage | None = None
        self.learning_rate = learning_rate
        self.schedule, self.desired_kl = schedule, desired_kl
        self.clip_param, self.gamma, self.lam = clip_param, gamma, lam
        self.num_learning_epochs, self.num_mini_batches = num_learning_epochs, num_mini_batches
        self.value_loss_coef, self.entropy_coef, self.max_grad_norm = value_loss_coef, entropy_coef, max_grad_norm
        self.use_clipped_value_loss = use_clipped_value_loss
        self.normalize_advantage_per_mini_batch = normalize_advantage_per_mini_batch
        self._t = {}
        self._flat_grad: torch.Tensor | None = None
        self._flat_adam = None
        use_flat_adam = on_gpu and bool(unused.get("fused_adam", True))
        if self.dist.world_size > 1:
            if not use_flat_adam:
                self._make_flat_grad_bucket()
            self.broadcast_parameters()
        if use_flat_adam:
            from .flat_adam import FlatAdam

            self._flat_adam = FlatAdam(self.optimizer)
            self._flat_grad = self._flat_adam.flat_g

    def _make_flat_grad_bucket(self) -> None:
        params = [p for p in self.actor_critic.parameters() if p.requires_grad]
        total = sum(p.numel() for p in params)
        self._flat_grad = torch.zeros(total, device=params[0].device, dtype=params[0].dtype)
        off = 0
        for p in params:
            p.grad = self._flat_grad[off:off + p.numel()].view_as(p)
            off += p.numel()

    def broadcast_parameters(self) -> None:
        for t in list(self.actor_critic.parameters()) + list(self.actor_critic.buffers()):
            self.dist.broadcast_(t.data, src=0)

    def init_storage(self, num_envs, num_transitions_per_env, actor_obs_shape, critic_obs_shape, action_shape,
                     obs_dtype: torch.dtype = torch.float32) -> None:
        self.storage = RolloutStorage(num_envs, num_transitions_per_env, actor_obs_shape[0], critic_obs_shape[0],
                                      action_shape[0], self.device, obs_dtype=obs_dtype)

    def test_mode(self) -> None:
        self.actor_critic.eval()

    def train_mode(self) -> None:
        self.actor_critic.train()

    def act(self, obs: torch.Tensor, critic_obs: torch.Tensor) -> torch.Tensor:
        ac, t = self.actor_critic, self._t
        if getattr(ac, "is_recurrent", False):
            t["hidden"] = tuple(None if h is None else (tuple(x.clone() for x in h) if isinstance(h, tuple) else h.clone())
                                for h in ac.get_hidden_states())
        t["actions"] = ac.act(obs).detach()
        t["values"] = ac.evaluate(critic_obs).detach()
        t["log_prob"] = ac.get_actions_log_prob(t["actions"]).detach()
        t["mu"] = ac.action_mean.detach()
        t["sigma"] = ac.action_std.detach()
        t["obs"], t["critic_obs"] = obs, critic_obs
        return t["actions"]

    def process_env_step(self, rewards: torch.Tensor, dones: torch.Tensor, infos: dict) -> None:
        t = self._t
        rew = rewards.clone()
        if "time_outs" in infos:
            rew += self.gamma * torch.squeeze(t["values"] * infos["time_outs"].unsqueeze(1).to(self.device), 1)
        self.storage.add(t["obs"], t["critic_obs"], t["actions"], rew, dones, t["values"], t["log_prob"], t["mu"], t["sigma"],
                         hidden_states=t.get("hidden"))
        self._t = {}
        self.actor_critic.reset(dones)

    def compute_returns(self, last_critic_obs: torch.Tensor) -> None:
        last_values = self.actor_critic.evaluate(last_critic_obs).detach()
        self.storage.compute_returns(last_values, self.gamma, self.lam,
                                     normalize_advantage=not self.normalize_advantage_per_mini_batch, dist=self.dist)

    def _fused_loss_ok(self, b) -> bool:
        ac = self.actor_critic
        st = self.storage
        return (self.fused_loss and st.observations.is_cuda and type(ac) is ActorCritic and getattr(ac, "noise_std_type", "scalar") == "scalar"
                and st.actions.shape[-1] <= 16)

    def _packed_pair(self):
        if not self.packed_forward:
            return None
        if self._pair is None:
            from .mlp import PackedPair, describe

            ac = self.actor_critic
            self._pair = False
            if describe(ac.actor) is not None and describe(ac.critic) is not None:
                try:
                    self._pair = PackedPair(ac.actor, ac.critic)
                except ValueError:
                    self._pair = False
        return self._pair or None

    def _flat_storage(self):
        st = self.storage
        f = lambda t: t.flatten(0, 1)
        small = [f(t).contiguous() for t in (st.actions, st.actions_log_prob, st.advantages, st.returns, st.values, st.mu, st.sigma)]
        return f(st.observations), f(st.privileged_observations), small

    def _fused_update(self):
        from .fused_loss import fused_ppo_loss

        ac, st = self.actor_critic, self.storage
        obs, cobs, small = self._flat_storage()
        stats = torch.zeros(3, device=obs.device)
        adaptive = self.desired_kl is not None and self.schedule == "adaptive"
        pair = self._packed_pair()
        if pair is not None and self._flat_adam is not None and self.direct_update and ac.std.requires_grad:
            return self._direct_update(pair)
        if pair is not None:
            pair.arm_domain_check()
        for idx in st.mini_batch_indices(self.num_mini_batches, self.num_learning_epochs):
            o, co = obs[idx], cobs[idx]
            if o.dtype != torch.float32:
                o, co = o.float(), co.float()
            mu, value = pair(o, co) if pair is not None else (ac.actor(o), ac.critic(co))
            loss, surrogate_loss, value_loss, ent, kl_mean = fused_ppo_loss(
                mu, ac.std, value, *small, self.clip_param, self.value_loss_coef, self.entropy_coef,
                self.use_clipped_value_loss, idx=idx)
            kl_handle = self.dist.all_reduce_mean_begin(kl_mean.detach().clone()) if adaptive else None
            self._zero_grad()
            loss.backward()
            if adaptive:
                self._apply_kl(self.dist.all_reduce_mean_end(kl_handle), reduced=True)
            self._optim_step()
            stats = stats + torch.stack((value_loss, surrogate_loss, ent.detach()))
        n = self.num_learning_epochs * self.num_mini_batches
        sv, ss, se = (stats / n).tolist()
        if pair is not None and pair.domain_violated():
            self._warn_mlp_domain()
        st.clear()
        return sv, ss, se, None, None

    def _direct_update(self, pair, split_buckets: bool = True):
        ac, st, fa = self.actor_critic, self.storage, self._flat_adam
        obs, cobs, small = self._flat_storage()
        small = [t.view(-1) if t.shape[-1] == 1 else t for t in small]
        dev = obs.device
        adaptive = self.desired_kl is not None and self.schedule == "adaptive"
        a_dim = small[0].shape[1]
        state = torch.zeros(4, device=dev)
        state[0] = self.learning_rate
        lr_dev, stats = state[:1], state[1:]
        grad_of = fa.grad_views()
        std_c = ac.std.detach()
        pair.arm_domain_check()
        n_steps = 0
        critic_at = fa.offset_of(next(iter(ac.critic.parameters())))
        two_buckets = split_buckets and 0 < critic_at < self._flat_grad.numel()
        perm, m = st.mini_batch_permutation(self.num_mini_batches)
        perm_o, perm_co = obs[perm], cobs[perm]
        if perm_o.dtype != torch.float32:
            perm_o, perm_co = perm_o.float(), perm_co.float()
        split_o = (pair.split_rows(perm_o), pair.split_rows(perm_co)) if pair._fused_backward_possible(perm_o[:m], perm_co[:m]) else None
        for step_i in range(self.num_learning_epochs * self.num_mini_batches):
            i = step_i % self.num_mini_batches
            idx = perm[i * m:(i + 1) * m]
            o, co = perm_o[i * m:(i + 1) * m], perm_co[i * m:(i + 1) * m]
            xs = (split_o[0][i * m:(i + 1) * m], split_o[1][i * m:(i + 1) * m]) if split_o is not None else None
            (mu, value), acts = pair.forward_raw(o, co)
            dmu = torch.empty_like(mu)
            dvalue = torch.empty(m, 1, device=dev, dtype=torch.float32)
            acc = torch.empty(24, device=dev, dtype=torch.float32)
            out = torch.empty(24, device=dev, dtype=torch.float32)
            stream = _abi.stream(dev)
            _abi.call("lt_ppo_loss", mu, std_c, value, *small, idx, m, a_dim, float(self.clip_param), float(self.value_loss_coef),
                      float(self.entropy_coef), int(bool(self.use_clipped_value_loss)), dmu, dvalue, acc, out, stream)
            kl = None
            if adaptive:
                kl = out[4:5]
                if self.dist.world_size > 1:
                    kl = self.dist.all_reduce_mean_(kl.clone())
            _abi.call("lt_ppo_lr_rule", kl, float(self.desired_kl or 0.0), 1e-5, 1e-2, 1.5, lr_dev, stats, out, grad_of[ac.std], a_dim, stream)
            if self.dist.world_size > 1 and two_buckets:
                handles = []
                pair.backward_raw(o, co, acts, dmu, dvalue, grad_of, xs, after_first=lambda: handles.append(self.dist.all_reduce_mean_begin(self._flat_grad[:critic_at])),
                                  dy_amax=(acc[20:21], acc[21:22]))
                handles.append(self.dist.all_reduce_mean_begin(self._flat_grad[critic_at:] if handles else self._flat_grad))
                for h in handles:
                    self.dist.all_reduce_mean_end(h)
            else:
                pair.backward_raw(o, co, acts, dmu, dvalue, grad_of, xs, dy_amax=(acc[20:21], acc[21:22]))
                if self.dist.world_size > 1:
                    self.dist.all_reduce_mean_(self._flat_grad)
            fa.step_dev(self.max_grad_norm, lr_dev)
            n_steps += 1
        sat = pair.saturated()
        lr, sv, ss, se, nsat = torch.cat((state, sat if sat is not None else state[:0].new_zeros(1))).tolist()
        if nsat > 0:
            import warnings

            sat.zero_()
            warnings.warn(f"lt_mlp_backward_pair: {int(nsat)} workgroup-layers of the gradient chain reached the f16 image's bound "
                          "(a gradient grew by more than 500x through the layers): those rows were saturated; set LT_FUSED_BACKWARD=0 "
                          "to run the chain as f32 library GEMMs")
        self.learning_rate = lr
        for group in self.optimizer.param_groups:
            group["lr"] = lr
        if pair.domain_violated():
            self._warn_mlp_domain()
        st.clear()
        return sv / n_steps, ss / n_steps, se / n_steps, None, None

    def _warn_mlp_domain(self) -> None:
        import warnings

        self.mlp_domain_violations = getattr(self, "mlp_domain_violations", 0) + 1
        warnings.warn("an observation or hidden activation reached the MLP kernel's saturation bound (|x| >= LT_MLP_INPUT_CLAMP, "
                      "include/lt_env.h): the fused forward computes MLP(clamp(x)) there, unlike the fp32 reference; "
                      "construct PPO(..., packed_forward=False) and FusedRollout(..., use_packed_mlp=False) to run the fp32 GEMM path")

    def _adapt_learning_rate(self, mu, sigma, old_mu, old_sigma) -> None:
        with torch.inference_mode():
            kl = torch.sum(torch.log(sigma / old_sigma + 1.0e-5)
                           + (torch.square(old_sigma) + torch.square(old_mu - mu)) / (2.0 * torch.square(sigma)) - 0.5, dim=-1)
            self._apply_kl(torch.mean(kl))

    def _apply_kl(self, kl_mean, reduced: bool = False) -> None:
        with torch.inference_mode():
            if self.dist.world_size > 1 and not reduced:
                kl_mean = self.dist.all_reduce_mean_(kl_mean.clone())
            kl_mean = float(kl_mean)
        if kl_mean > self.desired_kl * 2.0:
            self.learning_rate = max(1e-5, self.learning_rate / 1.5)
        elif self.desired_kl / 2.0 > kl_mean > 0.0:
            self.learning_rate = min(1e-2, self.learning_rate * 1.5)
        for group in self.optimizer.param_groups:
            group["lr"] = self.learning_rate

    def update(self):
        if self.fused_recurrent_update:
            return self._recurrent_update()
        return self._eager_update()

    def _recurrent_update_unsupported(self) -> str | None:
        from .memory_seq import unsupported
        from .modules import ActorCriticRecurrent

        ac = self.actor_critic
        if type(ac) is not ActorCriticRecurrent:
            return f"the policy is a {type(ac).__name__}: only a plain ActorCriticRecurrent is served"
        st = getattr(self, "storage", None)
        return unsupported(ac.memory_a, ac.memory_c, *((None, None) if st is None else (st.observations, st.privileged_observations)),
                           gru_memories=self.fused_gru_memories)

    def _recurrent_update(self):
        why = self._recurrent_update_unsupported()
        if why is not None:
            raise ValueError(f"fused_recurrent_update: {why}")
        from .memory_seq import memory_rollout_sequence

        ac, st = self.actor_critic, self.storage
        if st.saved_hidden_states_a is None or st.saved_hidden_states_c is None:
            raise ValueError("fused_recurrent_update: the storage holds no saved hidden states (no rollout of a recurrent policy filled it)")
        T, N = st.num_steps, st.num_envs
        per = N // self.num_mini_batches
        dones = st.dones.view(T, N)
        adaptive = self.desired_kl is not None and self.schedule == "adaptive"
        fused = (self.fused_loss and st.observations.is_cuda and getattr(ac, "noise_std_type", "scalar") == "scalar" and st.actions.shape[-1] <= 16)
        if fused:
            from .fused_loss import fused_ppo_loss
        blocks = []
        for i in range(self.num_mini_batches):
            sl = (slice(None), slice(i * per, (i + 1) * per))
            blocks.append((sl, st.observations[sl].contiguous(), st.privileged_observations[sl].contiguous()))
        stats = torch.zeros(3, device=st.observations.device, dtype=st.values.dtype)
        for _ in range(self.num_learning_epochs):
            for sl, obs, cobs in blocks:
                hc_a = tuple(h[0][sl] for h in st.saved_hidden_states_a)
                hc_c = tuple(h[0][sl] for h in st.saved_hidden_states_c)
                out_a, out_c = memory_rollout_sequence(ac.memory_a, ac.memory_c, obs, cobs, dones[sl], hc_a, hc_c,
                                                       gru_memories=self.fused_gru_memories)
                adv = st.advantages[sl]
                if self.normalize_advantage_per_mini_batch:
                    with torch.no_grad():
                        adv = (adv - adv.mean()) / (adv.std() + 1e-8)
                old_mu, old_sigma, old_values, returns = st.mu[sl], st.sigma[sl], st.values[sl], st.returns[sl]
                if fused:
                    f = lambda t: t.reshape(T * per, -1)
                    loss, surrogate_loss, value_loss, ent, kl_mean = fused_ppo_loss(
                        ac.actor(out_a.view(T * per, -1)), ac.std, ac.critic(out_c.view(T * per, -1)), f(st.actions[sl]),
                        f(st.actions_log_prob[sl]), f(adv), f(returns), f(old_values), f(old_mu), f(old_sigma), self.clip_param,
                        self.value_loss_coef, self.entropy_coef, self.use_clipped_value_loss)
                    if adaptive:
                        self._apply_kl(kl_mean)
                    ent = ent.detach()
                else:
                    ac.update_distribution(out_a)
                    log_prob = ac.get_actions_log_prob(st.actions[sl])
                    value = ac.critic(out_c)
                    mu, sigma, ent = ac.action_mean, ac.action_std, ac.entropy.mean()
                    if adaptive:
                        self._adapt_learning_rate(mu, sigma, old_mu, old_sigma)
                    ratio = torch.exp(log_prob - torch.squeeze(st.actions_log_prob[sl]))
                    a = torch.squeeze(adv)
                    surrogate_loss = torch.max(-a * ratio, -a * torch.clamp(ratio, 1.0 - self.clip_param, 1.0 + self.clip_param)).mean()
                    if self.use_clipped_value_loss:
                        clipped = old_values + (value - old_values).clamp(-self.clip_param, self.clip_param)
                        value_loss = torch.max((value - returns).pow(2), (clipped - returns).pow(2)).mean()
                    else:
                        value_loss = (returns - value).pow(2).mean()
                    loss = surrogate_loss + self.value_loss_coef * value_loss - self.entropy_coef * ent
                self._zero_grad()
                loss.backward()
                self._optim_step()
                stats = stats + torch.stack((value_loss.detach(), surrogate_loss.detach(), ent.detach())).to(stats.dtype)
        n = self.num_learning_epochs * self.num_mini_batches
        sv, ss, se = (stats / n).tolist()
        st.clear()
        return sv, ss, se, None, None

    def _eager_update(self):
        ac = self.actor_critic
        sum_value = sum_surr = sum_ent = 0.0
        stats = None
        recurrent = getattr(ac, "is_recurrent", False)
        if not recurrent and not self.normalize_advantage_per_mini_batch and self._fused_loss_ok(None):
            return self._fused_update()
        batches = (self.storage.recurrent_mini_batches(self.num_mini_batches, self.num_learning_epochs) if recurrent
                   else self.storage.mini_batches(self.num_mini_batches, self.num_learning_epochs))
        for raw in batches:
            if recurrent:
                from .storage import Batch

                b, (hid_a, hid_c), masks = Batch(*raw[:9]), raw[9], raw[10]
            else:
                b, hid_a, hid_c, masks = raw, None, None, None
            adv = b.advantages
            if self.normalize_advantage_per_mini_batch:
                with torch.no_grad():
                    adv = (adv - adv.mean()) / (adv.std() + 1e-8)
            if self._fused_loss_ok(b):
                from .fused_loss import fused_ppo_loss

                loss, surrogate_loss, value_loss, ent, kl_mean = fused_ppo_loss(
                    ac.actor(b.obs), ac.std, ac.critic(b.critic_obs), b.actions, b.log_prob, adv, b.returns, b.values, b.mu, b.sigma,
                    self.clip_param, self.value_loss_coef, self.entropy_coef, self.use_clipped_value_loss)
                if self.desired_kl is not None and self.schedule == "adaptive":
                    self._apply_kl(kl_mean)
                if stats is None:
                    stats = torch.zeros(3, device=loss.device)
                self._zero_grad()
                loss.backward()
                self._optim_step()
                stats = stats + torch.stack((value_loss, surrogate_loss, ent.detach()))
                continue
            if recurrent:
                ac.act(b.obs, masks=masks, hidden_states=hid_a)
                log_prob = ac.get_actions_log_prob(b.actions)
                value = ac.evaluate(b.critic_obs, masks=masks, hidden_states=hid_c)
            else:
                ac.act(b.obs)
                log_prob = ac.get_actions_log_prob(b.actions)
                value = ac.evaluate(b.critic_obs)
            mu, sigma, entropy = ac.action_mean, ac.action_std, ac.entropy
            if self.desired_kl is not None and self.schedule == "adaptive":
                self._adapt_learning_rate(mu, sigma, b.mu, b.sigma)
            ratio = torch.exp(log_prob - torch.squeeze(b.log_prob))
            a = torch.squeeze(adv)
            surrogate_loss = torch.max(-a * ratio, -a * torch.clamp(ratio, 1.0 - self.clip_param, 1.0 + self.clip_param)).mean()
            if self.use_clipped_value_loss:
                clipped = b.values + (value - b.values).clamp(-self.clip_param, self.clip_param)
                value_loss = torch.max((value - b.returns).pow(2), (clipped - b.returns).pow(2)).mean()
            else:
                value_loss = (b.returns - value).pow(2).mean()
            loss = surrogate_loss + self.value_loss_coef * value_loss - self.entropy_coef * entropy.mean()
            self._zero_grad()
            loss.backward()
            self._optim_step()
            sum_value += value_loss.item()
            sum_surr += surrogate_loss.item()
            sum_ent += entropy.mean().item()
        n = self.num_learning_epochs * self.num_mini_batches
        if stats is not None:
            sv, ss, se = stats.tolist()
            sum_value, sum_surr, sum_ent = sum_value + sv, sum_surr + ss, sum_ent + se
        self.storage.clear()
        return sum_value / n, sum_surr / n, sum_ent / n, None, None

    def _zero_grad(self) -> None:
        if self._flat_adam is not None:
            self._flat_adam.zero_grad()
        elif self._flat_grad is not None:
            self._flat_grad.zero_()
        else:
            self.optimizer.zero_grad()

    def _optim_step(self) -> None:
        if self._flat_adam is not None:
            self._flat_adam.gather_grads()
        if self.dist.world_size > 1:
            self.dist.all_reduce_mean_(self._flat_grad)
        if self._flat_adam is not None:
            self._flat_adam.step(self.max_grad_norm, gathered=True)
        else:
            nn.utils.clip_grad_norm_(self.actor_critic.parameters(), self.max_grad_norm)
            self.optimizer.step()
```

Measured before the change: 68.38 million.

## Fold PPO loss, finalize and LR rule into one kernel; pair head and wgrad launches

Adds a single-launch PPO loss step kernel that computes the per-row loss, reduces it across blocks with a last-block ticket, and then runs the finalize and adaptive-LR rule, replacing three separate launches. The small rollout tensors are pre-permuted once per update so the kernel reads them contiguously without index gathers. The two nets' head weight-gradient launches are paired into one grid, and same-shaped hidden-layer wgrad launches of actor and critic are paired into one kernel. The aim is to cut kernel-launch and sync overhead in the minibatch loop, at the cost of a cross-block atomic reduction and an extra gather of the small tensors.

New measurement: 68.50 million (median of 2 runs). No clear change (+0.2%).

```diff
diff --git a/include/lt_ppo_step.h b/include/lt_ppo_step.h
--- /dev/null
+++ b/include/lt_ppo_step.h
@@ -0,0 +1,28 @@
+#ifndef LT_PPO_STEP_H
+#define LT_PPO_STEP_H
+
+#include <stdint.h>
+
+#ifdef __cplusplus
+extern "C" {
+#endif
+
+int lt_ppo_loss_step(const float* mu, const float* std, const float* value, const float* actions, const float* old_logp, const float* adv,
+                     const float* returns, const float* old_values, const float* old_mu, const float* old_sigma, const int64_t* idx, int64_t M,
+                     int A, float clip, float value_loss_coef, float entropy_coef, int use_clipped_value_loss, float* dmu, float* dvalue,
+                     float* acc, float* out, float* ws, int apply_lr_rule, const float* kl_override, float desired_kl, float lr_min,
+                     float lr_max, float factor, float* lr, float* stats, float* dstd_out, void* stream);
+int lt_ppo_loss_step_rows(void);
+int64_t lt_ppo_loss_step_ws_floats(int64_t M);
+
+int lt_head_wgrad_pair(const float* dy0, const float* x0, int n0, int k0, float* ws0, const float* dy1, const float* x1, int n1, int k1,
+                       float* ws1, int x_split, int64_t M, void* stream);
+
+int lt_wgrad_pair(const float* dz0, const float* dz_scale0, const float* x0, const float* amax_blocks0, float* slabs0, float* db_slabs0,
+                  const float* dz1, const float* dz_scale1, const float* x1, const float* amax_blocks1, float* slabs1, float* db_slabs1,
+                  int dz_split, int x_split, int64_t M, int N, int K, int nblk_amax, void* stream);
+
+#ifdef __cplusplus
+}
+#endif
+#endif
diff --git a/locotouch_amd/_abi.py b/locotouch_amd/_abi.py
--- a/locotouch_amd/_abi.py
+++ b/locotouch_amd/_abi.py
@@ -18,6 +18,7 @@
 MEMORY_SEQ_HEADER = os.path.join(REPO, "include", "lt_memory_seq.h")
 MEMORY_GRU_HEADER = os.path.join(REPO, "include", "lt_memory_gru.h")
 POLICY_HEADER = os.path.join(REPO, "include", "lt_policy.h")
+PPO_STEP_HEADER = os.path.join(REPO, "include", "lt_ppo_step.h")
 LIB_PATH = os.environ.get("LOCOTOUCH_AMD_LIB", os.path.join(_HERE, "_lib", "liblocotouch_env.so"))
 
 _SCALARS = {"int": ctypes.c_int, "int32_t": ctypes.c_int32, "int64_t": ctypes.c_int64, "uint8_t": ctypes.c_uint8,
@@ -206,6 +207,17 @@
     raise ImportError("_abi.POLICY_VALUE_QUERIES does not match include/lt_policy.h, or an entry point there returns no int or repeats "
                       "one of another header")
 
+PPO_STEP_SIGNATURES = parse_header(open(PPO_STEP_HEADER).read())[2]
+PPO_STEP_VALUE_QUERIES = frozenset({"lt_ppo_loss_step_rows", "lt_ppo_loss_step_ws_floats"})
+if (not PPO_STEP_VALUE_QUERIES <= set(PPO_STEP_SIGNATURES)
+        or any(r is not ctypes.c_int for n, (r, _) in PPO_STEP_SIGNATURES.items() if n not in PPO_STEP_VALUE_QUERIES)
+        or set(PPO_STEP_SIGNATURES) & (set(EXPORTS) | set(OBS_NORM_SIGNATURES) | set(STUDENT_SIGNATURES) | set(COLLECT_SIGNATURES)
+                                       | set(LEDGER_SIGNATURES) | set(CNN_TRAIN_SIGNATURES) | set(BC_SIGNATURES) | set(LSTM_SIGNATURES)
+                                       | set(MEMORY_SIGNATURES) | set(MEMORY_SEQ_SIGNATURES) | set(MEMORY_GRU_SIGNATURES)
+                                       | set(POLICY_SIGNATURES))):
+    raise ImportError("_abi.PPO_STEP_VALUE_QUERIES does not match include/lt_ppo_step.h, or an entry point there returns no status or "
+                      "repeats one of another header")
+
 _lib = None
 _calls: dict = {}
 
@@ -220,11 +232,12 @@
     lib = ctypes.CDLL(LIB_PATH)
     for name, (restype, argtypes) in {**SIGNATURES, **OBS_NORM_SIGNATURES, **STUDENT_SIGNATURES, **COLLECT_SIGNATURES, **LEDGER_SIGNATURES,
                                       **CNN_TRAIN_SIGNATURES, **BC_SIGNATURES, **LSTM_SIGNATURES, **MEMORY_SIGNATURES,
-                                      **MEMORY_SEQ_SIGNATURES, **MEMORY_GRU_SIGNATURES, **POLICY_SIGNATURES}.items():
+                                      **MEMORY_SEQ_SIGNATURES, **MEMORY_GRU_SIGNATURES, **POLICY_SIGNATURES, **PPO_STEP_SIGNATURES}.items():
         fn = getattr(lib, name)
         fn.restype, fn.argtypes = restype, argtypes
         if (name not in VALUE_QUERIES and name not in STUDENT_VALUE_QUERIES and name not in CNN_TRAIN_VALUE_QUERIES
-                and name not in MEMORY_SEQ_VALUE_QUERIES and name not in MEMORY_GRU_VALUE_QUERIES and name not in POLICY_VALUE_QUERIES):
+                and name not in MEMORY_SEQ_VALUE_QUERIES and name not in MEMORY_GRU_VALUE_QUERIES and name not in POLICY_VALUE_QUERIES
+                and name not in PPO_STEP_VALUE_QUERIES):
             _calls[name] = (fn, [ptr if t is ctypes.c_void_p else _ref if issubclass(t, ctypes._Pointer) and issubclass(t._type_, ctypes.Structure)
                                  else None for t in argtypes])
     if lib.lt_cfg_sizeof() != ctypes.sizeof(LtCfg):
@@ -261,7 +274,7 @@
         fn, conv = _calls[name]
     except KeyError:
         if (name in VALUE_QUERIES or name in STUDENT_VALUE_QUERIES or name in CNN_TRAIN_VALUE_QUERIES or name in MEMORY_SEQ_VALUE_QUERIES
-                or name in MEMORY_GRU_VALUE_QUERIES or name in POLICY_VALUE_QUERIES):
+                or name in MEMORY_GRU_VALUE_QUERIES or name in POLICY_VALUE_QUERIES or name in PPO_STEP_VALUE_QUERIES):
             raise TypeError(f"{name} returns a value, not a status: call load().{name}(...)") from None
         if _lib is not None:
             raise
diff --git a/locotouch_amd/csrc/lt_ppo.hip b/locotouch_amd/csrc/lt_ppo.hip
--- a/locotouch_amd/csrc/lt_ppo.hip
+++ b/locotouch_amd/csrc/lt_ppo.hip
@@ -4,24 +4,23 @@
 
 #include "lt_env.h"
 #include "lt_internal.h"
+#include "lt_ppo_step.h"
 
 namespace {
 
 constexpr int MAX_A = 16;
 constexpr float kHalfLog2Pi = 0.91893853320467274178f;
 
-__global__ __launch_bounds__(256) void lt_ppo_loss_kernel(const float* __restrict__ mu, const float* __restrict__ stdp, const float* __restrict__ value,
-                                                          const float* __restrict__ actions, const float* __restrict__ old_logp,
-                                                          const float* __restrict__ adv, const float* __restrict__ returns,
-                                                          const float* __restrict__ old_values, const float* __restrict__ old_mu,
-                                                          const float* __restrict__ old_sigma, const long long* __restrict__ idx,
-                                                          long long M, int A, float clip, float vcoef, int clipped_value,
-                                                          float* __restrict__ dmu, float* __restrict__ dvalue, float* __restrict__ acc) {
-  const long long row = (long long)blockIdx.x * 256 + threadIdx.x;
+__device__ __forceinline__ void ppo_loss_row(const float* __restrict__ mu, const float* __restrict__ stdp, const float* __restrict__ value,
+                                             const float* __restrict__ actions, const float* __restrict__ old_logp,
+                                             const float* __restrict__ adv, const float* __restrict__ returns,
+                                             const float* __restrict__ old_values, const float* __restrict__ old_mu,
+                                             const float* __restrict__ old_sigma, const long long* __restrict__ idx, long long row,
+                                             long long M, int A, float clip, float vcoef, int clipped_value, float* __restrict__ dmu,
+                                             float* __restrict__ dvalue, float (&part)[4 + MAX_A], float& amax_mu, float& amax_v) {
   const bool ok = row < M;
   const long long src = (ok && idx) ? idx[row] : row;
-  float part[4 + MAX_A];
-  float amax_mu = 0.f, amax_v = 0.f;
+  amax_mu = 0.f; amax_v = 0.f;
 #pragma unroll
   for (int i = 0; i < 4 + MAX_A; ++i) part[i] = 0.f;
   if (ok) {
@@ -78,6 +77,20 @@
     part[1] = vl;
     part[2] = kl;
   }
+}
+
+__global__ __launch_bounds__(256) void lt_ppo_loss_kernel(const float* __restrict__ mu, const float* __restrict__ stdp, const float* __restrict__ value,
+                                                          const float* __restrict__ actions, const float* __restrict__ old_logp,
+                                                          const float* __restrict__ adv, const float* __restrict__ returns,
+                                                          const float* __restrict__ old_values, const float* __restrict__ old_mu,
+                                                          const float* __restrict__ old_sigma, const long long* __restrict__ idx,
+                                                          long long M, int A, float clip, float vcoef, int clipped_value,
+                                                          float* __restrict__ dmu, float* __restrict__ dvalue, float* __restrict__ acc) {
+  const long long row = (long long)blockIdx.x * 256 + threadIdx.x;
+  float part[4 + MAX_A];
+  float amax_mu, amax_v;
+  ppo_loss_row(mu, stdp, value, actions, old_logp, adv, returns, old_values, old_mu, old_sigma, idx, row, M, A, clip, vcoef, clipped_value, dmu, dvalue,
+               part, amax_mu, amax_v);
   __shared__ float red[4][4 + MAX_A];
   const int lane = threadIdx.x & 63, wave = threadIdx.x >> 6;
 #pragma unroll
@@ -104,21 +117,29 @@
   }
 }
 
-__global__ __launch_bounds__(64) void lt_ppo_finalize_kernel(const float* __restrict__ acc, const float* __restrict__ stdp, int A, float inv_m,
-                                                             float vcoef, float ecoef, float* __restrict__ out) {
+__device__ __forceinline__ void ppo_finalize(const float* acc, const float* __restrict__ stdp, int A, float inv_m, float vcoef, float ecoef,
+                                             float* __restrict__ out, float& dstd, float (&sc)[5]) {
   const int a = threadIdx.x;
   float e = 0.f;
   if (a < A) {
     const float sg = stdp[a];
     e = 0.5f + kHalfLog2Pi + logf(sg);
-    out[8 + a] = acc[4 + a] - ecoef / sg;
+    dstd = acc[4 + a] - ecoef / sg;
+    out[8 + a] = dstd;
   }
   for (int off = 32; off > 0; off >>= 1) e += __shfl_xor(e, off, 64);
   if (a == 0) {
     const float surr = acc[0] * inv_m, vl = acc[1] * inv_m;
-    out[0] = surr + vcoef * vl - ecoef * e;
-    out[1] = surr; out[2] = vl; out[3] = e; out[4] = acc[2] * inv_m;
-  }
+    sc[0] = surr + vcoef * vl - ecoef * e;
+    sc[1] = surr; sc[2] = vl; sc[3] = e; sc[4] = acc[2] * inv_m;
+    out[0] = sc[0]; out[1] = sc[1]; out[2] = sc[2]; out[3] = sc[3]; out[4] = sc[4];
+  }
+}
+
+__global__ __launch_bounds__(64) void lt_ppo_finalize_kernel(const float* __restrict__ acc, const float* __restrict__ stdp, int A, float inv_m,
+                                                             float vcoef, float ecoef, float* __restrict__ out) {
+  float dstd = 0.f, sc[5];
+  ppo_finalize(acc, stdp, A, inv_m, vcoef, ecoef, out, dstd, sc);
 }
 
 constexpr int EB_ROWS = 48;
@@ -244,8 +265,8 @@
 constexpr int HW_ROWS = 96, HW_MAX_N = 16;
 
 template <int NN>
-__global__ __launch_bounds__(256) void lt_head_wgrad_kernel(const float* __restrict__ dy, const float* __restrict__ x, int x_split, long long M, int n, int k,
-                                                            float* __restrict__ ws) {
+__device__ __forceinline__ void head_wgrad_body(const float* __restrict__ dy, const float* __restrict__ x, int x_split, long long M, int n, int k,
+                                                float* __restrict__ ws) {
   const int k4 = k >> 2, lanes = 256 / k4;
   const int c4 = threadIdx.x % k4, rl = threadIdx.x / k4;
   const long long r0 = (long long)blockIdx.x * HW_ROWS;
@@ -307,6 +328,24 @@
     for (int l = 1; l < lanes; ++l) t += redb[l * NN + threadIdx.x];
     out[(size_t)n * k + threadIdx.x] = t;
   }
+}
+
+template <int NN>
+__global__ __launch_bounds__(256) void lt_head_wgrad_kernel(const float* __restrict__ dy, const float* __restrict__ x, int x_split, long long M, int n, int k,
+                                                            float* __restrict__ ws) {
+  head_wgrad_body<NN>(dy, x, x_split, M, n, k, ws);
+}
+
+struct HeadPair {
+  const float* dy[2];
+  const float* x[2];
+  float* ws[2];
+  int n[2], k[2];
+};
+template <int NN0, int NN1>
+__global__ __launch_bounds__(256) void lt_head_wgrad_pair_kernel(const HeadPair p, int x_split, long long M) {
+  if (blockIdx.y == 0) head_wgrad_body<NN0>(p.dy[0], p.x[0], x_split, M, p.n[0], p.k[0], p.ws[0]);
+  else head_wgrad_body<NN1>(p.dy[1], p.x[1], x_split, M, p.n[1], p.k[1], p.ws[1]);
 }
 
 __global__ __launch_bounds__(256) void lt_gae_kernel(const float* __restrict__ rewards, const unsigned char* __restrict__ dones,
@@ -378,11 +417,8 @@
   }
 }
 
-__global__ __launch_bounds__(64) void lt_ppo_lr_rule_kernel(const float* __restrict__ kl_mean, float desired, float lr_min, float lr_max, float factor,
-                                                            float* __restrict__ lr, float* __restrict__ stats, const float* __restrict__ scalars,
-                                                            float* __restrict__ dstd_out, int A) {
-  if (dstd_out && scalars && (int)threadIdx.x < A) dstd_out[threadIdx.x] = scalars[8 + threadIdx.x];
-  if (threadIdx.x != 0) return;
+__device__ __forceinline__ void ppo_lr_rule_lane0(const float* kl_mean, float desired, float lr_min, float lr_max, float factor, float* lr, float* stats,
+                                                  const float* scalars) {
   if (kl_mean && desired > 0.f) {
 #pragma clang fp reciprocal(off)
     const float kl = *kl_mean;
@@ -394,6 +430,123 @@
   if (stats && scalars) { stats[0] += scalars[2]; stats[1] += scalars[1]; stats[2] += scalars[3]; }
 }
 
+__global__ __launch_bounds__(64) void lt_ppo_lr_rule_kernel(const float* __restrict__ kl_mean, float desired, float lr_min, float lr_max, float factor,
+                                                            float* __restrict__ lr, float* __restrict__ stats, const float* __restrict__ scalars,
+                                                            float* __restrict__ dstd_out, int A) {
+  if (dstd_out && scalars && (int)threadIdx.x < A) dstd_out[threadIdx.x] = scalars[8 + threadIdx.x];
+  if (threadIdx.x != 0) return;
+  ppo_lr_rule_lane0(kl_mean, desired, lr_min, lr_max, factor, lr, stats, scalars);
+}
+
+constexpr int LS_ROWS = 128, LS_WAVES = LS_ROWS / 64, LS_STRIDE = 24, LS_HEAD = 32, LS_LANES = LS_ROWS / 8;
+
+struct LossStepRule {
+  int apply;
+  const float* kl_in;
+  float desired, lr_min, lr_max, factor;
+  float* lr;
+  float* stats;
+  float* dstd_out;
+};
+
+__global__ __launch_bounds__(LS_ROWS) void lt_ppo_loss_step_kernel(const float* __restrict__ mu, const float* __restrict__ stdp, const float* __restrict__ value,
+                                                                   const float* __restrict__ actions, const float* __restrict__ old_logp,
+                                                                   const float* __restrict__ adv, const float* __restrict__ returns,
+                                                                   const float* __restrict__ old_values, const float* __restrict__ old_mu,
+                                                                   const float* __restrict__ old_sigma, const long long* __restrict__ idx,
+                                                                   long long M, int A, float clip, float vcoef, float ecoef, int clipped_value,
+                                                                   float* __restrict__ dmu, float* __restrict__ dvalue, float* __restrict__ acc,
+                                                                   float* __restrict__ out, float* ws, float inv_m, const LossStepRule rule) {
+  const long long row = (long long)blockIdx.x * LS_ROWS + threadIdx.x;
+  float part[4 + MAX_A];
+  float amax_mu, amax_v;
+  ppo_loss_row(mu, stdp, value, actions, old_logp, adv, returns, old_values, old_mu, old_sigma, idx, row, M, A, clip, vcoef, clipped_value, dmu, dvalue,
+               part, amax_mu, amax_v);
+  __shared__ float red[LS_WAVES][LS_STRIDE];
+  __shared__ float4 fin[LS_LANES][6];
+  __shared__ float s_acc[LS_STRIDE];
+  __shared__ int s_last;
+  const int lane = threadIdx.x & 63, wave = threadIdx.x >> 6;
+#pragma unroll
+  for (int i = 0; i < 4 + MAX_A; ++i) {
+    float v = part[i];
+#pragma unroll
+    for (int off = 32; off > 0; off >>= 1) v += __shfl_xor(v, off, 64);
+    if (lane == 0) red[wave][i] = v;
+  }
+#pragma unroll
+  for (int off = 32; off > 0; off >>= 1) {
+    amax_mu = fmaxf(amax_mu, __shfl_xor(amax_mu, off, 64));
+    amax_v = fmaxf(amax_v, __shfl_xor(amax_v, off, 64));
+  }
+  if (lane == 0) { red[wave][20] = amax_mu; red[wave][21] = amax_v; red[wave][22] = 0.f; red[wave][23] = 0.f; }
+  __syncthreads();
+  if (wave == 0) {
+    if (lane < LS_STRIDE) {
+      float v = red[0][lane];
+#pragma unroll
+      for (int w = 1; w < LS_WAVES; ++w) v = lane < 20 ? v + red[w][lane] : fmaxf(v, red[w][lane]);
+      ws[LS_HEAD + (long long)blockIdx.x * LS_STRIDE + lane] = v;
+    }
+    asm volatile("s_waitcnt vmcnt(0)" ::: "memory");
+    if (lane == 0) {
+      __threadfence();
+      asm volatile("s_waitcnt vmcnt(0)" ::: "memory");
+      const unsigned ticket = atomicAdd((unsigned*)ws, 1u);
+      const int last = ticket == gridDim.x - 1u;
+      if (last) {
+        __threadfence();
+        asm volatile("s_waitcnt vmcnt(0)" ::: "memory");
+      }
+      s_last = last;
+    }
+  }
+  __syncthreads();
+  if (!s_last) return;
+  {
+    const int nblk = (int)gridDim.x, q = threadIdx.x & 7, l = threadIdx.x >> 3;
+    const int per = (nblk + LS_LANES - 1) / LS_LANES;
+    const int b0 = min(l * per, nblk), b1 = min(b0 + per, nblk);
+    float4 s = {0.f, 0.f, 0.f, 0.f};
+    if (q < 6) {
+      const float4* rows = (const float4*)(ws + LS_HEAD);
+#pragma unroll 4
+      for (int b = b0; b < b1; ++b) {
+        const float4 v = rows[(long long)b * 6 + q];
+        s.x = q == 5 ? fmaxf(s.x, v.x) : s.x + v.x;
+        s.y = q == 5 ? fmaxf(s.y, v.y) : s.y + v.y;
+        s.z += v.z; s.w += v.w;
+      }
+      fin[l][q] = s;
+    }
+  }
+  __syncthreads();
+  if (threadIdx.x < 6) {
+    const int q = threadIdx.x;
+    float4 t = fin[0][q];
+    for (int l = 1; l < LS_LANES; ++l) {
+      const float4 v = fin[l][q];
+      t.x = q == 5 ? fmaxf(t.x, v.x) : t.x + v.x;
+      t.y = q == 5 ? fmaxf(t.y, v.y) : t.y + v.y;
+      t.z += v.z; t.w += v.w;
+    }
+    s_acc[4 * q] = t.x; s_acc[4 * q + 1] = t.y; s_acc[4 * q + 2] = t.z; s_acc[4 * q + 3] = t.w;
+  }
+  __syncthreads();
+  if (wave != 0) return;
+  if (lane < LS_STRIDE) acc[lane] = s_acc[lane];
+  float dstd = 0.f, sc[5];
+  ppo_finalize(s_acc, stdp, A, inv_m, vcoef, ecoef, out, dstd, sc);
+  if (rule.apply) {
+    if (rule.dstd_out && lane < A) rule.dstd_out[lane] = dstd;
+    if (lane == 0) {
+      const float kl = rule.kl_in ? *rule.kl_in : sc[4];
+      ppo_lr_rule_lane0(&kl, rule.desired, rule.lr_min, rule.lr_max, rule.factor, rule.lr, rule.stats, sc);
+    }
+  }
+  if (lane == 0) __hip_atomic_store((unsigned*)ws, 0u, __ATOMIC_RELAXED, __HIP_MEMORY_SCOPE_AGENT);
+}
+
 }
 
 extern "C" int lt_ppo_lr_rule(const float* kl_mean, float desired_kl, float lr_min, float lr_max, float factor, float* lr, float* stats,
@@ -427,6 +580,12 @@
   return LT_OK;
 }
 
+static int head_nn(int n) { return n <= 1 ? 1 : (n <= 4 ? 4 : (n <= 8 ? 8 : (n <= 12 ? 12 : 16))); }
+static size_t head_lds_bytes(int nn, int k) {
+  const int k4 = k / 4, lanes = 256 / k4;
+  return (size_t)lanes * nn * k4 * 16 + (size_t)lanes * nn * 4;
+}
+
 extern "C" int64_t lt_head_wgrad_ws_floats(int64_t M, int n, int k) { return ((M + HW_ROWS - 1) / HW_ROWS) * ((int64_t)n * k + HW_MAX_N); }
 
 extern "C" int lt_head_wgrad(const float* dy, const float* x, int x_split, int64_t M, int n, int k, float* dw, float* db, float* ws, void* stream) {
@@ -434,9 +593,9 @@
     lt_set_error("lt_head_wgrad: invalid argument (1 <= n <= 16, k a multiple of 4, 4 <= k <= 1024)");
     return LT_EINVAL;
   }
-  const int nblk = (int)((M + HW_ROWS - 1) / HW_ROWS), k4 = k / 4, lanes = 256 / k4;
-  const int nn = n <= 1 ? 1 : (n <= 4 ? 4 : (n <= 8 ? 8 : (n <= 12 ? 12 : 16)));
-  const size_t lds = (size_t)lanes * nn * k4 * 16 + (size_t)lanes * nn * 4;
+  const int nblk = (int)((M + HW_ROWS - 1) / HW_ROWS);
+  const int nn = head_nn(n);
+  const size_t lds = head_lds_bytes(nn, k);
   if (const int e = lt_ensure_dynamic_lds((const void*)lt_head_wgrad_kernel<16>, 72 * 1024)) {
     lt_set_error(hipGetErrorString((hipError_t)e));
     return LT_EHIP;
@@ -551,3 +710,83 @@
   if (e != hipSuccess) { lt_set_error(hipGetErrorString(e)); return LT_EHIP; }
   return LT_OK;
 }
+
+extern "C" int lt_ppo_loss_step_rows(void) { return LS_ROWS; }
+extern "C" int64_t lt_ppo_loss_step_ws_floats(int64_t M) { return LS_HEAD + ((M + LS_ROWS - 1) / LS_ROWS) * LS_STRIDE; }
+
+extern "C" int lt_ppo_loss_step(const float* mu, const float* stdp, const float* value, const float* actions, const float* old_logp, const float* adv,
+                                const float* returns, const float* old_values, const float* old_mu, const float* old_sigma, const int64_t* idx,
+                                int64_t M, int A, float clip, float value_loss_coef, float entropy_coef, int use_clipped_value_loss, float* dmu,
+                                float* dvalue, float* acc, float* out, float* ws, int apply_lr_rule, const float* kl_override, float desired_kl,
+                                float lr_min, float lr_max, float factor, float* lr, float* stats, float* dstd_out, void* stream) {
+  if (!mu || !stdp || !value || !actions || !old_logp || !adv || !returns || !old_values || !old_mu || !old_sigma || !dmu || !dvalue || !acc ||
+      !out || !ws || (reinterpret_cast<uintptr_t>(ws) & 15) || M < 1 || A < 1 || A > MAX_A || (M + LS_ROWS - 1) / LS_ROWS > 0x7fffffff) {
+    lt_set_error("lt_ppo_loss_step: invalid argument (1 <= num_actions <= 16; out and a 16-byte aligned ws are required)");
+    return LT_EINVAL;
+  }
+  if (apply_lr_rule && (!lr || factor <= 1.f)) { lt_set_error("lt_ppo_loss_step: invalid argument (the rule needs lr and factor > 1)"); return LT_EINVAL; }
+  LossStepRule rule = {};
+  if (apply_lr_rule) {
+    rule.apply = 1; rule.kl_in = kl_override; rule.desired = desired_kl; rule.lr_min = lr_min; rule.lr_max = lr_max; rule.factor = factor;
+    rule.lr = lr; rule.stats = stats; rule.dstd_out = dstd_out;
+  }
+  hipLaunchKernelGGL(lt_ppo_loss_step_kernel, dim3((unsigned)((M + LS_ROWS - 1) / LS_ROWS)), dim3(LS_ROWS), 0, (hipStream_t)stream, mu, stdp, value, actions,
+                     old_logp, adv, returns, old_values, old_mu, old_sigma, (const long long*)idx, (long long)M, A, clip, value_loss_coef, entropy_coef,
+                     use_clipped_value_loss, dmu, dvalue, acc, out, ws, 1.f / (float)M, rule);
+  const hipError_t e = hipGetLastError();
+  if (e != hipSuccess) { lt_set_error(hipGetErrorString(e)); return LT_EHIP; }
+  return LT_OK;
+}
+
+namespace {
+template <int NN0, int NN1>
+int launch_head_pair(const HeadPair& p, int x_split, long long M, size_t lds, hipStream_t st) {
+  if (lds > 60 * 1024)
+    if (const int e = lt_ensure_dynamic_lds((const void*)lt_head_wgrad_pair_kernel<NN0, NN1>, 72 * 1024)) return e;
+  hipLaunchKernelGGL((lt_head_wgrad_pair_kernel<NN0, NN1>), dim3((unsigned)((M + HW_ROWS - 1) / HW_ROWS), 2), dim3(256), lds, st, p, x_split, M);
+  return 0;
+}
+template <int NN0>
+int launch_head_pair0(int nn1, const HeadPair& p, int x_split, long long M, size_t lds, hipStream_t st) {
+  switch (nn1) {
+    case 1: return launch_head_pair<NN0, 1>(p, x_split, M, lds, st);
+    case 4: return launch_head_pair<NN0, 4>(p, x_split, M, lds, st);
+    case 8: return launch_head_pair<NN0, 8>(p, x_split, M, lds, st);
+    case 12: return launch_head_pair<NN0, 12>(p, x_split, M, lds, st);
+    default: return launch_head_pair<NN0, 16>(p, x_split, M, lds, st);
+  }
+}
+}
+
+extern "C" int lt_head_wgrad_pair(const float* dy0, const float* x0, int n0, int k0, float* ws0, const float* dy1, const float* x1, int n1, int k1,
+                                  float* ws1, int x_split, int64_t M, void* stream) {
+  const auto bad = [](const float* dy, const float* x, const float* ws, int n, int k) {
+    return !dy || !x || !ws || n < 1 || n > HW_MAX_N || k < 4 || (k & 3) || k > 1024;
+  };
+  if (M < 1 || bad(dy0, x0, ws0, n0, k0) || bad(dy1, x1, ws1, n1, k1)) {
+    lt_set_error("lt_head_wgrad_pair: invalid argument (per head: 1 <= n <= 16, k a multiple of 4, 4 <= k <= 1024)");
+    return LT_EINVAL;
+  }
+  const int nn0 = head_nn(n0), nn1 = head_nn(n1);
+  const size_t l0 = head_lds_bytes(nn0, k0), l1 = head_lds_bytes(nn1, k1), lds = l0 > l1 ? l0 : l1;
+  if (lds > 72 * 1024) {
+    lt_set_error("lt_head_wgrad_pair: n * k too large for one block's LDS partials");
+    return LT_EINVAL;
+  }
+  HeadPair p;
+  p.dy[0] = dy0; p.dy[1] = dy1; p.x[0] = x0; p.x[1] = x1; p.ws[0] = ws0; p.ws[1] = ws1;
+  p.n[0] = n0; p.n[1] = n1; p.k[0] = k0; p.k[1] = k1;
+  hipStream_t st = (hipStream_t)stream;
+  int rc;
+  switch (nn0) {
+    case 1: rc = launch_head_pair0<1>(nn1, p, x_split, (long long)M, lds, st); break;
+    case 4: rc = launch_head_pair0<4>(nn1, p, x_split, (long long)M, lds, st); break;
+    case 8: rc = launch_head_pair0<8>(nn1, p, x_split, (long long)M, lds, st); break;
+    case 12: rc = launch_head_pair0<12>(nn1, p, x_split, (long long)M, lds, st); break;
+    default: rc = launch_head_pair0<16>(nn1, p, x_split, (long long)M, lds, st); break;
+  }
+  if (rc) { lt_set_error(hipGetErrorString((hipError_t)rc)); return LT_EHIP; }
+  const hipError_t e = hipGetLastError();
+  if (e != hipSuccess) { lt_set_error(hipGetErrorString(e)); return LT_EHIP; }
+  return LT_OK;
+}
diff --git a/locotouch_amd/csrc/lt_wgrad.hip b/locotouch_amd/csrc/lt_wgrad.hip
--- a/locotouch_amd/csrc/lt_wgrad.hip
+++ b/locotouch_amd/csrc/lt_wgrad.hip
@@ -3,6 +3,7 @@
 
 #include "lt_env.h"
 #include "lt_internal.h"
+#include "lt_ppo_step.h"
 
 namespace {
 
@@ -59,7 +60,7 @@
 
 constexpr int WG_WAVES = 4;
 template <bool AS, bool XS>
-__global__ __launch_bounds__(64 * WG_WAVES, 2) void lt_wgrad_kernel(const WgradArgs a) {
+__device__ __forceinline__ void wgrad_body(const WgradArgs& a) {
   __shared__ f32x4 s_tile[WG_WAVES - 1][TA * TB + 1][64];
   const int lane = threadIdx.x & 63;
   const int wave = __builtin_amdgcn_readfirstlane((int)threadIdx.x >> 6);
@@ -194,6 +195,17 @@
     }
 }
 
+template <bool AS, bool XS>
+__global__ __launch_bounds__(64 * WG_WAVES, 2) void lt_wgrad_kernel(const WgradArgs a) {
+  wgrad_body<AS, XS>(a);
+}
+
+template <bool AS, bool XS>
+__global__ __launch_bounds__(64 * WG_WAVES, 2) void lt_wgrad_pair_kernel(const WgradArgs a0, const WgradArgs a1) {
+  const WgradArgs a = blockIdx.y == 0 ? a0 : a1;
+  wgrad_body<AS, XS>(a);
+}
+
 int pick_splits(long long M, int tiles) {
   const long long steps = (M + 31) / 32;
   long long s = 512 / tiles;
@@ -234,6 +246,34 @@
   return LT_OK;
 }
 
+extern "C" int lt_wgrad_pair(const float* dz0, const float* dz_scale0, const float* x0, const float* amax_blocks0, float* slabs0, float* db_slabs0,
+                             const float* dz1, const float* dz_scale1, const float* x1, const float* amax_blocks1, float* slabs1, float* db_slabs1,
+                             int dz_split, int x_split, int64_t M, int N, int K, int nblk_amax, void* stream) {
+  if (!dz0 || !x0 || !slabs0 || !dz1 || !x1 || !slabs1 || M < 1 || N < 4 || K < 4 || (N & 3) || (K & 3) || (!amax_blocks0 != !amax_blocks1) ||
+      (amax_blocks0 && nblk_amax < 1) || (!db_slabs0 != !db_slabs1) || (long long)M * (N > K ? N : K) * 4 >= (1ll << 32)) {
+    lt_set_error("lt_wgrad_pair: invalid argument (N and K multiples of 4, each operand below 4 GiB, amax_blocks and db_slabs for both problems or neither)");
+    return LT_EINVAL;
+  }
+  if (dz_split && (!dz_scale0 || !dz_scale1)) { lt_set_error("lt_wgrad_pair: a split dz needs its scale"); return LT_EINVAL; }
+  WgradArgs a;
+  a.dz = dz0; a.x = x0; a.M = M; a.N = N; a.K = K;
+  a.amax = amax_blocks0; a.nblk_amax = amax_blocks0 ? nblk_amax : 0;
+  a.slabs = slabs0; a.db = db_slabs0; a.x_split = x_split != 0; a.dz_split = dz_split != 0; a.dz_scale = dz_scale0;
+  a.tiles_n = (N + 16 * TA - 1) / (16 * TA);
+  a.tiles_k = (K + 16 * TB - 1) / (16 * TB);
+  a.splits = pick_splits((long long)M, a.tiles_n * a.tiles_k);
+  WgradArgs b = a;
+  b.dz = dz1; b.x = x1; b.amax = amax_blocks1; b.slabs = slabs1; b.db = db_slabs1; b.dz_scale = dz_scale1;
+  const dim3 grid((unsigned)((a.tiles_n * a.tiles_k * a.splits + 7) / 8 * 8), 2);
+  if (a.dz_split && a.x_split) hipLaunchKernelGGL((lt_wgrad_pair_kernel<true, true>), grid, dim3(64 * WG_WAVES), 0, (hipStream_t)stream, a, b);
+  else if (a.x_split) hipLaunchKernelGGL((lt_wgrad_pair_kernel<false, true>), grid, dim3(64 * WG_WAVES), 0, (hipStream_t)stream, a, b);
+  else if (a.dz_split) hipLaunchKernelGGL((lt_wgrad_pair_kernel<true, false>), grid, dim3(64 * WG_WAVES), 0, (hipStream_t)stream, a, b);
+  else hipLaunchKernelGGL((lt_wgrad_pair_kernel<false, false>), grid, dim3(64 * WG_WAVES), 0, (hipStream_t)stream, a, b);
+  const hipError_t e = hipGetLastError();
+  if (e != hipSuccess) { lt_set_error(hipGetErrorString(e)); return LT_EHIP; }
+  return LT_OK;
+}
+
 namespace {
 __global__ __launch_bounds__(256) void lt_split_rows_kernel(const float* __restrict__ x, unsigned* __restrict__ out, long long n4) {
   typedef unsigned u32x4 __attribute__((ext_vector_type(4)));
diff --git a/locotouch_amd/rl/mlp.py b/locotouch_amd/rl/mlp.py
--- a/locotouch_amd/rl/mlp.py
+++ b/locotouch_amd/rl/mlp.py
@@ -327,7 +327,7 @@
     def _fused_backward_ok(self, x0, x1, dy0, dy1) -> bool:
         return self._fused_backward_possible(x0, x1) and dy0.dtype == torch.float32 and dy1.dtype == torch.float32
 
-    def _backward_fused(self, x0, x1, acts, dy0, dy1, grad_of, sums, x_split_rows=None, after_first=None, dy_amax=None) -> None:
+    def _backward_fused(self, x0, x1, acts, dy0, dy1, grad_of, sums, x_split_rows=None, after_first=None, dy_amax=None, fold=False) -> None:
         lib = _abi.load()
         stream = _abi.stream()
         m = x0.shape[0]
@@ -345,33 +345,59 @@
         nblk = lib.lt_mlp_backward_blocks(ctypes.byref(nets[0].desc), ctypes.byref(nets[1].desc), m)
         dzs, amaxs, arrs = [], [], []
         per_net = (SumJobs(), SumJobs()) if after_first is not None else (sums, sums)
+        fold = bool(fold) and after_first is None
+        heads = []
         for k, net in enumerate(nets):
             if not self._bpacked_fresh:
                 net.pack_backward()
             L = len(net.linears)
             n, kk = dys[k].shape[1], acts[k][L - 2].shape[1]
             ws = torch.empty(lib.lt_head_wgrad_ws_floats(m, n, kk), device=dev, dtype=torch.float32)
-            _abi.call("lt_head_wgrad", dys[k], acts[k][L - 2], asp, m, n, kk, None, None, ws, stream)
+            heads.append((dys[k], acts[k][L - 2], n, kk, ws))
+            if not fold:
+                _abi.call("lt_head_wgrad", dys[k], acts[k][L - 2], asp, m, n, kk, None, None, ws, stream)
             per_net[k].add(ws, lib.lt_head_wgrad_nblk(m), n * kk + 16, n * kk + n, n * kk, grad_of[net.linears[L - 1].weight], grad_of[net.linears[L - 1].bias])
             dz = [torch.empty_like(a) for a in acts[k]]
             am = torch.empty(L - 1, nblk, device=dev, dtype=torch.float32)
             dzs.append(dz)
             amaxs.append(am)
             arrs.append((_abi.ptr_array(acts[k]), _abi.ptr_array(dz), _abi.ptr_array([am[l] for l in range(L - 1)])))
+        if fold:
+            _abi.call("lt_head_wgrad_pair", *heads[0], *heads[1], asp, m, stream)
         dzsp = int(dy_amax is not None)
         scales = torch.empty(2, device=dev, dtype=torch.float32)
         in_amax = dy_amax if dzsp else (None, None)
         _abi.call("lt_mlp_backward_pair", nets[0].desc, nets[0].bpacked, dys[0], *arrs[0], nets[1].desc, nets[1].bpacked, dys[1], *arrs[1],
                   m, asp, in_amax[0], in_amax[1], dzsp, scales, self.sat, stream)
+        paired = {}
+        if fold:
+            for d in range(min(len(n_.linears) for n_ in nets) - 1):
+                l0, l1 = len(nets[0].linears) - 2 - d, len(nets[1].linears) - 2 - d
+                shape = lambda k, l: (dzs[k][l].shape[1], (acts[k][l - 1] if l > 0 else xs[k]).shape[1], int(l > 0))
+                if shape(0, l0) == shape(1, l1):
+                    paired[(0, l0)] = (1, l1)
+        launched = {}
         for k, net in enumerate(nets):
             for l in range(len(net.linears) - 2, -1, -1):
                 inp = acts[k][l - 1] if l > 0 else xs[k]
                 dz = dzs[k][l]
                 n, kk = dz.shape[1], inp.shape[1]
                 sp = lib.lt_wgrad_splits(m, n, kk)
-                slabs = torch.empty(sp * n * kk + sp * n, device=dev, dtype=torch.float32)
-                dbs = slabs[sp * n * kk:]
-                _abi.call("lt_wgrad", dz, dzsp, scales[k:k + 1], inp, asp if l > 0 else xsp, m, n, kk, amaxs[k][l], nblk, slabs, dbs, stream)
+                if (k, l) in launched:
+                    slabs = launched[(k, l)]
+                    dbs = slabs[sp * n * kk:]
+                else:
+                    slabs = torch.empty(sp * n * kk + sp * n, device=dev, dtype=torch.float32)
+                    dbs = slabs[sp * n * kk:]
+                    if (k, l) in paired:
+                        k1, l1 = paired[(k, l)]
+                        slabs1 = torch.empty_like(slabs)
+                        launched[(k1, l1)] = slabs1
+                        _abi.call("lt_wgrad_pair", dz, scales[k:k + 1], inp, amaxs[k][l], slabs, dbs,
+                                  dzs[k1][l1], scales[k1:k1 + 1], acts[k1][l1 - 1] if l1 > 0 else xs[k1], amaxs[k1][l1], slabs1, slabs1[sp * n * kk:],
+                                  dzsp, asp if l > 0 else xsp, m, n, kk, nblk, stream)
+                    else:
+                        _abi.call("lt_wgrad", dz, dzsp, scales[k:k + 1], inp, asp if l > 0 else xsp, m, n, kk, amaxs[k][l], nblk, slabs, dbs, stream)
                 gw = grad_of[net.linears[l].weight]
                 if kk != gw.shape[1]:
                     pad = torch.empty(n, kk, device=dev, dtype=torch.float32)
@@ -390,10 +416,10 @@
     def saturated(self) -> torch.Tensor | None:
         return self.sat
 
-    def backward_raw(self, x0, x1, acts, dy0, dy1, grad_of, x_split_rows=None, after_first=None, dy_amax=None) -> None:
+    def backward_raw(self, x0, x1, acts, dy0, dy1, grad_of, x_split_rows=None, after_first=None, dy_amax=None, fold=False) -> None:
         sums = SumJobs()
         if self._fused_backward_ok(x0, x1, dy0, dy1):
-            self._backward_fused(x0, x1, acts, dy0, dy1, grad_of, sums, x_split_rows, after_first, dy_amax)
+            self._backward_fused(x0, x1, acts, dy0, dy1, grad_of, sums, x_split_rows, after_first, dy_amax, fold)
             sums.launch()
             return
         if self.acts_split:
diff --git a/locotouch_amd/rl/ppo.py b/locotouch_amd/rl/ppo.py
--- a/locotouch_amd/rl/ppo.py
+++ b/locotouch_amd/rl/ppo.py
@@ -21,6 +21,7 @@
         self.fused_loss = on_gpu and bool(unused.get("fused_loss", True))
         self.packed_forward = on_gpu and bool(unused.get("packed_forward", True))
         self.direct_update = on_gpu and bool(unused.get("direct_update", True))
+        self.fold_step = on_gpu and bool(unused.get("fold_step", True))
         self.fused_recurrent_update = bool(unused.get("fused_recurrent_update", False))
         self.fused_gru_memories = bool(unused.get("fused_gru_memories", False))
         if self.fused_recurrent_update:
@@ -189,6 +190,11 @@
         if perm_o.dtype != torch.float32:
             perm_o, perm_co = perm_o.float(), perm_co.float()
         split_o = (pair.split_rows(perm_o), pair.split_rows(perm_co)) if pair._fused_backward_possible(perm_o[:m], perm_co[:m]) else None
+        fold = self.fold_step and self.dist.world_size == 1
+        if fold:
+            small = [t[perm] for t in small]
+            lib = _abi.load()
+            loss_ws = torch.zeros(lib.lt_ppo_loss_step_ws_floats(m), device=dev, dtype=torch.float32)
         for step_i in range(self.num_learning_epochs * self.num_mini_batches):
             i = step_i % self.num_mini_batches
             idx = perm[i * m:(i + 1) * m]
@@ -200,6 +206,15 @@
             acc = torch.empty(24, device=dev, dtype=torch.float32)
             out = torch.empty(24, device=dev, dtype=torch.float32)
             stream = _abi.stream(dev)
+            if fold:
+                sm = [t[i * m:(i + 1) * m] for t in small]
+                _abi.call("lt_ppo_loss_step", mu, std_c, value, *sm, None, m, a_dim, float(self.clip_param), float(self.value_loss_coef),
+                          float(self.entropy_coef), int(bool(self.use_clipped_value_loss)), dmu, dvalue, acc, out, loss_ws,
+                          1, None, float(self.desired_kl or 0.0) if adaptive else 0.0, 1e-5, 1e-2, 1.5, lr_dev, stats, grad_of[ac.std], stream)
+                pair.backward_raw(o, co, acts, dmu, dvalue, grad_of, xs, dy_amax=(acc[20:21], acc[21:22]), fold=True)
+                fa.step_dev(self.max_grad_norm, lr_dev)
+                n_steps += 1
+                continue
             _abi.call("lt_ppo_loss", mu, std_c, value, *small, idx, m, a_dim, float(self.clip_param), float(self.value_loss_coef),
                       float(self.entropy_coef), int(bool(self.use_clipped_value_loss)), dmu, dvalue, acc, out, stream)
             kl = None
```
